# ML200/RoyalTracer-DX

Measured on AMD Instinct MI355X. Metric: Mrays/s + ms/frame at 1080p, 8-bounce Cornell Box, higher is better.
Workload: dtype f32; 1 GPU; cornell_1080p_64spp_8b; scene=generated: Cornell Box (32 triangles, 2 emissive), width=1920, height=1080, spp=64, max_bounces=8, nee_samples=1, rr_start=3, flags=1, triangles=32, parallelism=pixel-tiles/1, tile_size=64

## Files before the change

royaltracer-dx_amd/csrc/rtx_dev_common.hpp:

```cpp
#pragma once
#include "rtx_kernels.hpp"

namespace rtx {

constexpr int kBlock = 256;
constexpr uint32_t kMaxNee = 16;

__device__ __forceinline__ uint32_t lane_id() { return __builtin_amdgcn_mbcnt_hi(~0u, __builtin_amdgcn_mbcnt_lo(~0u, 0u)); }

__device__ __forceinline__ uint32_t block_push(bool pred, uint32_t* lds_counter) {
    const unsigned long long mask = __ballot(pred);
    const uint32_t cnt = (uint32_t)__popcll(mask);
    if (cnt == 0) return 0xFFFFFFFFu;
    const uint32_t prefix = __builtin_amdgcn_mbcnt_hi((uint32_t)(mask >> 32), __builtin_amdgcn_mbcnt_lo((uint32_t)mask, 0u));
    uint32_t base = 0;
    if (lane_id() == 0) base = atomicAdd(lds_counter, cnt);
    base = (uint32_t)__builtin_amdgcn_readfirstlane((int)base);
    return base + prefix;
}

__device__ __forceinline__ bool slot_to_pixel(const DevFrame& f, uint32_t pl, uint32_t& x, uint32_t& y) {
    const uint32_t ts2 = 2u * f.tile_shift;
    const uint32_t k = pl >> ts2, r = pl & ((1u << ts2) - 1u);
    uint32_t tx, ty;
    if (!shard_tile(f, k, tx, ty)) return false;
    const uint32_t bshift = f.tile_shift - 3u;
    const uint32_t blk = r >> 6, ln = r & 63u;
    const uint32_t bx = blk & ((1u << bshift) - 1u), by = blk >> bshift;
    x = (tx << f.tile_shift) + bx * 8u + (ln & 7u);
    y = (ty << f.tile_shift) + by * 8u + (ln >> 3);
    return x < f.width && y < f.height;
}

template <bool LIST> __device__ __forceinline__ uint32_t real_slot(const DevFrame& f, uint32_t v) {
    if constexpr (LIST) return f.list[v >> 8] * (uint32_t)kBlock + (v & 255u);
    else return v;
}
__device__ __forceinline__ bool chunk_image_index(const DevFrame& f, uint32_t lc, uint32_t& gi) {
    const uint32_t cs = 2u * f.tile_shift - 8u;
    uint32_t tx, ty;
    if (!shard_tile(f, lc >> cs, tx, ty)) return false;
    gi = ((ty * f.tiles_x + tx) << cs) | (lc & ((1u << cs) - 1u));
    return true;
}

__device__ __forceinline__ void primary_ray(const CameraGPU& cam, uint32_t W, uint32_t H, uint32_t x, uint32_t y, float jx, float jy, f3& o, f3& d) {
    const float dx = (((float)x + jx) / (float)W) * 2.0f - 1.0f;
    const float dy = (((float)y + jy) / (float)H) * 2.0f - 1.0f;
    const float* P = cam.projI; const float* Vi = cam.viewI;
    const float ndy = -dy;
    f3 tg = mk3(P[0] * dx + P[4] * ndy + P[8] + P[12], P[1] * dx + P[5] * ndy + P[9] + P[13], P[2] * dx + P[6] * ndy + P[10] + P[14]);
    d = normalize(xform_dir(Vi, tg));
    o = mk3(Vi[12], Vi[13], Vi[14]);
}

static_assert(sizeof(CameraGPU) == 64 * sizeof(float), "stage_camera copies one float per lane of the first wave");
__device__ __forceinline__ void stage_camera(CameraGPU& cam, const CameraGPU* __restrict__ cam_p) {
    if (threadIdx.x < 64) ((float*)&cam)[threadIdx.x] = ((const float*)cam_p)[threadIdx.x];
}

__device__ __forceinline__ bool dealt_chunk(const DevFrame& f, uint32_t k, uint32_t& row0, uint32_t nchunks, uint32_t& c) {
    const uint32_t nk = f.taper_levels ? taper_row_width(k, gridDim.x, f.taper_levels) : gridDim.x;
    uint32_t pos = blockIdx.x;
    if (f.taper_levels && blockIdx.x < nk) { pos += (k * 2654435761u) % nk; if (pos >= nk) pos -= nk; }
    c = row0 + pos;
    row0 += nk;
    return !(blockIdx.x >= nk || c >= nchunks);
}

}
```

royaltracer-dx_amd/csrc/rtx_k_bounce_small.hpp:

```cpp
#pragma once
#include "rtx_shade.hpp"

namespace rtx {

template <int WAVES, int HAVE_HIT, bool LAMBERT, bool RING>
__global__ __launch_bounds__(kBlock, WAVES) void k_bounce_small(DevScene sc, const SmallRecPair* __restrict__ small, DevFrame f_in, DevPaths p,
                                                         uint32_t bounce_first, uint32_t bounce_end,
                                                         uint32_t* __restrict__ queue_a, uint32_t* __restrict__ queue_b ,
                                                         uint32_t* __restrict__ qrows ,
                                                         uint32_t* __restrict__ srows ,
                                                         const uint32_t* __restrict__ order ,
                                                         const F4* __restrict__ prim_rec ) {
    extern __shared__ F4 lds[];
    __shared__ uint32_t s_cnt[1 + kMaxNee];
    DevFrame f = f_in;
    f.flags = LAMBERT ? (f_in.flags | 1u) : (f_in.flags & ~1u);
    const uint32_t qid = order ? order[blockIdx.x] : blockIdx.x;
#ifdef RTX_WAVE_CLOCK
    #define RTX_WAVE_STAMP_B(K) do { const uint32_t w_ = blockIdx.x * (kBlock / 64u) + (threadIdx.x >> 6); if (!HAVE_HIT && lane_id() == 0 && w_ < 65536u) g_wgt[2u * w_ + (K)] = __builtin_amdgcn_s_memrealtime(); } while (0)
    RTX_WAVE_STAMP_B(0u);
#endif
    __shared__ F4 s_sho[kBlock], s_shd[kBlock];
    __shared__ uint32_t s_shn[2];
    __shared__ uint8_t s_occ[kBlock];
    if (threadIdx.x <= kMaxNee) s_cnt[threadIdx.x] = 0;
    if (threadIdx.x < 2) s_shn[threadIdx.x] = 0;
#ifndef RTX_NO_SMALL_LDS_TABLES
    constexpr uint32_t kSmallLights = 32, kSmallMats = 16;
    __shared__ F4 s_lt[kSmallLights * 5]; __shared__ float s_ltcdf[kSmallLights]; __shared__ F4 s_mt[kSmallMats * 10];
    const bool lt_lds = sc.nlights && sc.nlights <= kSmallLights, mt_lds = sc.nmat && sc.nmat <= kSmallMats;
    if (lt_lds) { for (uint32_t i = threadIdx.x; i < sc.nlights * 5u; i += kBlock) s_lt[i] = ((const F4*)sc.lights)[i]; if (threadIdx.x < sc.nlights) s_ltcdf[threadIdx.x] = sc.cdf[threadIdx.x]; }
    if (mt_lds) for (uint32_t i = threadIdx.x; i < sc.nmat * 10u; i += kBlock) s_mt[i] = ((const F4*)sc.mats)[i];
    const MatGPU* mats = mt_lds ? (const MatGPU*)s_mt : sc.mats;
    const LightGPU* lds_lights = lt_lds ? (const LightGPU*)s_lt : nullptr; const float* lds_cdf = lt_lds ? s_ltcdf : nullptr;
#else
    const MatGPU* mats = sc.mats; const LightGPU* lds_lights = nullptr; const float* lds_cdf = nullptr;
#endif
    const uint32_t G = gridDim.x;
    uint32_t n = qrows[(size_t)bounce_first * G + qid];
    const uint32_t nee = sc.nlights ? f.nee_samples : 0u;
    const uint32_t nee1 = nee ? nee : 1u;
    const TraceLds L = stage_lds(sc, lds);
    __syncthreads();
    const size_t qb = (size_t)qid * f.qcap;
    uint32_t par = 0;
    constexpr uint32_t kRing = 512u;
    __shared__ uint32_t s_rpid[(HAVE_HIT || !RING) ? 1 : kRing];
    __shared__ F4 s_rhit[(HAVE_HIT || !RING) ? 1 : kRing];
    __shared__ uint32_t s_ring[1], s_rc[3];
    PF_BEGIN;
    for (uint32_t bounce = bounce_first; bounce < bounce_end; bounce++) {
    const bool last = (bounce + 1u == f.max_bounces);
    const float tmin = bounce_tmin(bounce);
    const uint32_t sbounce = HAVE_HIT == 2 ? 0u : bounce;
    const uint32_t* myq = ((bounce & 1u) ? queue_b : queue_a) + qb;
    uint32_t* mynext = ((bounce & 1u) ? queue_a : queue_b) + qb;
    if (!HAVE_HIT && RING) { if (threadIdx.x < 3) s_rc[threadIdx.x] = 0; if (threadIdx.x == 3) s_ring[0] = 0; __syncthreads(); }
    uint32_t next_in = 0;
    uint32_t prod = 0, rk = 0;
    for (uint32_t base = 0; (HAVE_HIT || !RING) ? base < n : true; base += kBlock) {
        PathState S; S.pid = 0; S.o = mk3(0, 0, 0); S.d = mk3(0, 0, 1); S.thr = mk3(0, 0, 0); S.prev_pdf = 1.0f; S.s0 = S.s1 = 0;
        float t = 0.0f, u = 0.0f, v = 0.0f; uint32_t prim = kMissPrim;
        bool active;
        PF_MARK(0);
        Surf sf; sf.mat = 0; sf.normal = mk3(0, 0, 1); sf.pos = mk3(0, 0, 0);
        if (HAVE_HIT == 2) {
            const uint32_t i = base + threadIdx.x;
            active = i < n;
            if (active) {
                S.pid = myq[i];
                const F4 e = p.hit[S.pid];
                const uint32_t pl = f2u(e.x);
                const F4 r0 = prim_rec[pl], r1 = prim_rec[(size_t)f.npl + pl], r2 = prim_rec[(size_t)2 * f.npl + pl], ro = prim_rec[(size_t)3 * f.npl];
                S.s0 = f2u(e.y); S.s1 = f2u(e.z);
                S.o = mk3(ro.x, ro.y, ro.z); S.d = mk3(r0.x, r0.y, r0.z); S.thr = mk3(1.0f, 1.0f, 1.0f); S.prev_pdf = 1.0f;
                sf.pos = mk3(r1.x, r1.y, r1.z); sf.normal = mk3(r2.x, r2.y, r2.z); sf.mat = f2u(r0.w); sf.near_hull = f2u(r1.w) != 0u;
                prim = 0u;
            }
        } else if (HAVE_HIT) {
            const uint32_t i = base + threadIdx.x;
            active = i < n;
            if (active) { S = load_path(p, myq[i]); const F4 h = p.hit[S.pid]; t = h.x; u = h.y; v = h.z; prim = f2u(h.w); }
        } else if (!RING) {
            const uint32_t i = base + threadIdx.x;
            active = i < n;
            if (active) S = load_path(p, myq[i]);
            traverse_small<false>(sc, small, L, S.o, S.d, tmin, active ? kTMax : 0.0f, t, u, v, prim, sc.nsmall, ~0ull, pf, 1);
        } else {
            while (next_in < n && prod - s_ring[0] < kBlock) {
                const uint32_t i = next_in + threadIdx.x;
                const bool act = i < n;
                uint32_t pid = 0; f3 ro = mk3(0, 0, 0), rd = mk3(0, 0, 1);
                if (act) { pid = myq[i]; const F4 a = p.ray_o[pid], b = p.ray_d[pid]; ro = mk3(a.x, a.y, a.z); rd = mk3(b.x, b.y, b.z); }
                float ht, hu, hv; uint32_t hp;
                traverse_small<false>(sc, small, L, ro, rd, tmin, act ? kTMax : 0.0f, ht, hu, hv, hp, sc.nsmall, ~0ull, pf, 1);
                const bool hit = act && hp != kMissPrim;
                const uint32_t slot = prod + block_push(hit, &s_rc[rk]);
                if (hit) { s_rpid[slot & (kRing - 1u)] = pid; s_rhit[slot & (kRing - 1u)] = {ht, hu, hv, u2f(hp)}; }
                next_in += kBlock;
                __syncthreads();
                prod += s_rc[rk];
                if (threadIdx.x == 0) s_rc[rk == 0u ? 2u : rk - 1u] = 0;
                rk = rk == 2u ? 0u : rk + 1u;
            }
            const uint32_t head = s_ring[0], avail = prod - head;
            if (avail == 0u) break;
            const uint32_t take = avail < (uint32_t)kBlock ? avail : (uint32_t)kBlock;
            active = threadIdx.x < take;
            if (active) {
                const uint32_t e = (head + threadIdx.x) & (kRing - 1u);
                S = load_path(p, s_rpid[e]);
                const F4 h = s_rhit[e]; t = h.x; u = h.y; v = h.z; prim = f2u(h.w);
            }
            __syncthreads();
            if (threadIdx.x == 0) s_ring[0] = head + take;
        }
        PF_MARK(2);
        bool shading = false;
        if (active && prim != kMissPrim) {
            PF_COUNT(3);
            if (HAVE_HIT != 2) sf = surface(sc, S.o, S.d, t, u, v, prim);
            if (sf.mat < sc.nmat) {
                const MatGPU& m = mats[sf.mat];
                if (m.Ke_len > 0.0f) add_emissive(sc, p, S, sf, m, sbounce, nee, HAVE_HIT != 0);
                else shading = true;
            } else if (HAVE_HIT) p.rad[S.pid] = {0.0f, 0.0f, 0.0f, 0.0f};
        }
        const f3 outgoing = -S.d, pos = sf.pos;
        const MatGPU* mp = mats + (shading ? sf.mat : 0u);
        f3 normal = sf.normal;
        const float eta_p = LAMBERT ? 0.0f : transmission_eta(*mp, f.flags, outgoing, normal);
        bool loaded = HAVE_HIT && shading; F4 radv = {0, 0, 0, 0};
        PF_MARK(3);
        for (uint32_t j = 0; j < nee; j++) {
            bool push = false;
            F4 so = {0, 0, 0, 0}, sd = {0, 0, 1, 0}; f3 con = mk3(0, 0, 0);
            if (shading) { PF_COUNT(4); push = nee_sample(sc, *mp, f.flags, nee, S, pos, normal, outgoing, so, sd, con, sf.near_hull, eta_p, nullptr, lds_cdf, lds_lights); }
            PF_MARK(4);
            const uint32_t slot = block_push(push, &s_shn[par]);
            if (push) { s_sho[slot] = so; s_shd[slot] = sd; }
            __syncthreads();
            PF_MARK(5);
            const uint32_t ns = s_shn[par];
            if ((threadIdx.x & ~63u) < ns) {
                const bool mine = threadIdx.x < ns;
                const F4 ro = mine ? s_sho[threadIdx.x] : F4{0, 0, 0, 0}, rd = mine ? s_shd[threadIdx.x] : F4{0, 0, 1, 0};
                float st_, su_, sv_; uint32_t sprim;
                const uint32_t nrec_sh = __builtin_amdgcn_ballot_w64(mine && ro.w < 0.0f) != 0ull ? sc.nsmall : sc.nsmall_occ;
                traverse_small<true>(sc, small, L, mk3(ro.x, ro.y, ro.z), mk3(rd.x, rd.y, rd.z), fabsf(ro.w), mine ? rd.w : 0.0f, st_, su_, sv_, sprim, nrec_sh, ~0ull, pf, 6);
                if (mine) s_occ[threadIdx.x] = sprim != kMissPrim ? 1 : 0;
            }
            PF_MARK(7);
            if (threadIdx.x == 0) { s_shn[par ^ 1u] = 0; s_cnt[1 + j] += ns; }
            __syncthreads();
            PF_MARK(8);
            if (push && !s_occ[slot]) {
                if (!loaded) { radv = p.rad[S.pid]; loaded = true; }
                radv.x = radv.x + con.x; radv.y = radv.y + con.y; radv.z = radv.z + con.z;
            }
            par ^= 1u;
        }
        if (loaded) p.rad[S.pid] = radv;
        bool alive = false;
        f3 smp = mk3(0, 0, 1); float P = 0.0f;
        if (shading && !last) { PF_COUNT(9); alive = bsdf_continue(*mp, f, sbounce, S, normal, outgoing, smp, P, eta_p); }
        if (alive) { PF_COUNT(10); store_path(p, S, pos, smp, P); }
        const uint32_t slot = block_push(alive, &s_cnt[0]);
        if (alive) mynext[slot] = S.pid;
        PF_MARK(9);
        if (!HAVE_HIT && RING) __syncthreads();
    }
    __syncthreads();
    n = s_cnt[0];
    if (threadIdx.x == 0) qrows[(size_t)(bounce + 1u) * G + qid] = n;
    if (threadIdx.x >= 1 && threadIdx.x <= nee) srows[((size_t)bounce * nee1 + (threadIdx.x - 1)) * G + qid] = s_cnt[threadIdx.x];
    __syncthreads();
    if (threadIdx.x <= kMaxNee) s_cnt[threadIdx.x] = 0;
    __syncthreads();
    }
    PF_FLUSH;
#ifdef RTX_WAVE_CLOCK
    RTX_WAVE_STAMP_B(1u);
#endif
}

}
```

royaltracer-dx_amd/csrc/rtx_k_film.hpp:

```cpp
#pragma once
#include "rtx_shade.hpp"

namespace rtx {

template <bool LIST>
__global__ __launch_bounds__(kBlock) void k_accumulate(DevFrame f, DevPaths p, F4* __restrict__ accum, AdaptState ad) {
    const uint32_t stride = gridDim.x * kBlock;
    for (uint32_t pl = blockIdx.x * kBlock + threadIdx.x; pl < f.npl; pl += stride) {
        uint32_t x, y;
        if constexpr (LIST) {
            uint32_t gi;
            if ((pl & 255u) == 0u && chunk_image_index(f, f.list[pl >> 8], gi)) ad.count[gi] = ad.count[gi] + f.batch_spp;
        }
        if (!slot_to_pixel(f, real_slot<LIST>(f, pl), x, y)) continue;
        F4 a = accum[(size_t)y * f.width + x];
        F4 h = {0.0f, 0.0f, 0.0f, 0.0f};
        if constexpr (LIST) h = ad.half[(size_t)y * f.width + x];
        for (uint32_t s = 0; s < f.batch_spp; s++) {
            const size_t pid = (size_t)s * f.npl + pl;
            F4 r = {0.0f, 0.0f, 0.0f, 0.0f};
            if (!p.hitmask || ((p.hitmask[pid >> 6] >> (pl & 63u)) & 1ull)) r = p.rad[pid];
            const f3 rv = mk3(r.x, r.y, r.z);
            if (finite3(rv)) {
                a.x = a.x + rv.x; a.y = a.y + rv.y; a.z = a.z + rv.z; a.w = a.w + 1.0f;
                if constexpr (LIST) if ((f.sample_first + s) & 1u) { h.x = h.x + rv.x; h.y = h.y + rv.y; h.z = h.z + rv.z; h.w = h.w + 1.0f; }
            }
        }
        accum[(size_t)y * f.width + x] = a;
        if constexpr (LIST) ad.half[(size_t)y * f.width + x] = h;
    }
}

__global__ __launch_bounds__(kBlock) void k_srgb8(const F4* __restrict__ accum, uint32_t npix, uint32_t* __restrict__ out) {
    const uint32_t i = blockIdx.x * kBlock + threadIdx.x;
    if (i >= npix) return;
    const F4 a = accum[i];
    const float cnt = maxf_(a.w, 1.0f);
    float c[3] = {a.x / cnt, a.y / cnt, a.z / cnt};
    if (is_nan(c[0]) || is_nan(c[1]) || is_nan(c[2])) { c[0] = 1.0f; c[1] = 0.0f; c[2] = 1.0f; }
    if (is_inf(c[0]) || is_inf(c[1]) || is_inf(c[2])) { c[0] = 0.0f; c[1] = 1.0f; c[2] = 1.0f; }
    uint32_t px = 0xFF000000u;
    for (int k = 0; k < 3; k++) {
        float v = c[k] <= 0.0031308f ? 12.92f * c[k] : 1.055f * pow_(c[k], 1.0f / 2.4f) - 0.055f;
        v = saturate(v);
        px |= ((uint32_t)(int)(v * 255.0f + 0.5f)) << (8 * k);
    }
    out[i] = px;
}

__device__ __forceinline__ uint32_t hash_colour(uint32_t id) {
    uint32_t h = id * 2654435761u + 0x9E3779B9u; h ^= h >> 15; h *= 0x85EBCA6Bu; h ^= h >> 13;
    return 0xFF000000u | (0x404040u + (h & 0x00BFBFBFu));
}
__device__ __forceinline__ uint32_t pack_rgb8(float r, float g, float b) {
    const float c[3] = {saturate(r), saturate(g), saturate(b)};
    uint32_t px = 0xFF000000u;
    for (int k = 0; k < 3; k++) px |= ((uint32_t)(int)(c[k] * 255.0f + 0.5f)) << (8 * k);
    return px;
}
__global__ __launch_bounds__(kBlock) void k_debug_layer(DevScene sc, const SmallRecPair* __restrict__ small, uint32_t width, uint32_t height, const CameraGPU* __restrict__ cam, uint32_t layer, uint32_t* __restrict__ out) {
    extern __shared__ F4 lds[];
    const TraceLds L = stage_lds(sc, lds);
    __syncthreads();
    const uint32_t stride = gridDim.x * kBlock;
    for (uint32_t i = blockIdx.x * kBlock + threadIdx.x; i < width * height; i += stride) {
        const uint32_t x = i % width, y = i / width;
        f3 o, d; primary_ray(*cam, width, height, x, y, 0.0f, 0.0f, o, d);
        float t, u, v; uint32_t prim;
        trace_ray<false>(sc, small, L, o, d, kTMinCam, kTMax, t, u, v, prim);
        uint32_t px = 0xFF000000u;
        if (prim != kMissPrim && layer >= 10u && layer <= 17u) {
            const Surf sf = surface(sc, o, d, t, u, v, prim);
            const bool hm = sf.mat < sc.nmat;
            const MatGPU& m = sc.mats[hm ? sf.mat : 0u];
            switch (layer) {
            case 10u: px = pack_rgb8(sf.normal.x * 0.5f + 0.5f, sf.normal.y * 0.5f + 0.5f, sf.normal.z * 0.5f + 0.5f); break;
            case 11u: { const float z = t / (1.0f + t); px = pack_rgb8(z, z, z); break; }
            case 12u: px = hash_colour(sf.mat); break;
            case 13u: px = hm ? pack_rgb8(m.Kd[0], m.Kd[1], m.Kd[2]) : px; break;
            case 14u: px = hash_colour(sf.inst + 0x51ED27u); break;
            case 15u: px = pack_rgb8(1.0f - u - v, u, v); break;
            case 16u: px = hm ? pack_rgb8(m.Ke[0] / (1.0f + m.Ke[0]), m.Ke[1] / (1.0f + m.Ke[1]), m.Ke[2] / (1.0f + m.Ke[2])) : px; break;
            default: px = hm ? pack_rgb8(m.Pr, m.Pm, m.alpha) : px; break;
            }
        }
        out[i] = px;
    }
}

__global__ __launch_bounds__(kBlock) void k_pack_tiles(DevFrame f, const F4* __restrict__ accum, F4* __restrict__ slab) {
    const uint32_t stride = gridDim.x * kBlock;
    for (uint32_t pl = blockIdx.x * kBlock + threadIdx.x; pl < f.npl; pl += stride) {
        uint32_t x, y;
        F4 v = {0, 0, 0, 0};
        if (slot_to_pixel(f, pl, x, y)) v = accum[(size_t)y * f.width + x];
        slab[pl] = v;
    }
}
__global__ __launch_bounds__(kBlock) void k_unpack_tiles(DevFrame f, uint32_t nshards, const F4* __restrict__ slabs, F4* __restrict__ accum) {
    const uint32_t stride = gridDim.x * kBlock;
    const uint32_t total = f.npl * nshards;
    for (uint32_t i = blockIdx.x * kBlock + threadIdx.x; i < total; i += stride) {
        DevFrame g = f; g.shard_rank = i / f.npl; g.shard_count = nshards;
        uint32_t x, y;
        if (slot_to_pixel(g, i - g.shard_rank * f.npl, x, y)) accum[(size_t)y * f.width + x] = slabs[i];
    }
}

}
```

royaltracer-dx_amd/csrc/rtx_k_raygen.hpp:

```cpp
#pragma once
#include "rtx_shade.hpp"

namespace rtx {

template <bool LIST>
__global__ __launch_bounds__(kBlock) void k_raygen(DevFrame f, DevPaths p, const CameraGPU* __restrict__ cam_p, uint32_t* __restrict__ queue, uint32_t* __restrict__ qcount, uint32_t compact) {
    __shared__ CameraGPU cam;
    __shared__ uint32_t s_n;
    stage_camera(cam, cam_p);
    if (threadIdx.x == 0) s_n = 0;
    __syncthreads();
    uint32_t* myq = queue + (size_t)blockIdx.x * f.qcap;
    const uint32_t nchunks = f.chunks_per_sample * f.batch_spp;
    for (uint32_t k = 0, row0 = 0, c; row0 < nchunks; k++) {
        if (!dealt_chunk(f, k, row0, nchunks, c)) continue;
        uint32_t sl = c / f.chunks_per_sample, cl = c - sl * f.chunks_per_sample;
        uint32_t pl = cl * kBlock + threadIdx.x;
        if (f.interleave) {
            const uint32_t sh = f.interleave, S = 1u << sh;
            const uint32_t per = S * f.chunks_per_sample, sg = c / per, r = c - sg * per;
            sl = sg * S + (threadIdx.x & (S - 1u));
            pl = r * (kBlock >> sh) + (threadIdx.x >> sh);
        }
        const uint32_t pid = sl * f.npl + pl;
        uint32_t x = 0, y = 0;
        const bool valid = slot_to_pixel(f, real_slot<LIST>(f, pl), x, y);
        const uint32_t slot = block_push(valid, &s_n);
        if (valid) {
            uint32_t s0, s1; seed_init(x, y, f.sample_first + sl, f.frame_seed, s0, s1);
            float jx = 0.0f, jy = 0.0f;
            if (f.flags & 2u) { jx = tea_next(s0, s1); jy = tea_next(s0, s1); }
            f3 o, d; primary_ray(cam, f.width, f.height, x, y, jx, jy, o, d);
            const uint32_t dst = compact ? blockIdx.x * f.qcap + slot : pid;
            p.ray_o[dst] = {o.x, o.y, o.z, u2f(s1)};
            p.ray_d[dst] = {d.x, d.y, d.z, 1.0f};
            p.thr[dst] = {1.0f, 1.0f, 1.0f, u2f(s0)};
            p.rad[pid] = {0.0f, 0.0f, 0.0f, 0.0f};
            myq[slot] = pid;
        }
    }
    __syncthreads();
    if (threadIdx.x == 0) qcount[blockIdx.x] = s_n;
}

__global__ __launch_bounds__(kBlock) void k_packet_masks(DevScene sc, DevFrame f, const CameraGPU* __restrict__ cam_p, unsigned long long* __restrict__ masks) {
    __shared__ CameraGPU cam;
    stage_camera(cam, cam_p);
    __syncthreads();
    const uint32_t blk = blockIdx.x * (kBlock / 64u) + (threadIdx.x >> 6);
    if (blk >= f.npl / 64u) return;
    uint32_t x = 0, y = 0;
    (void)slot_to_pixel(f, blk * 64u, x, y);
    const unsigned long long keep = packet_keep_mask(sc, cam, f, x & ~7u, y & ~7u);
    if (lane_id() == 0) masks[blk] = keep;
}

template <bool LIST>
__global__ __launch_bounds__(kBlock) void k_raygen_trace_small(DevScene sc, const SmallRecPair* __restrict__ small, DevFrame f, DevPaths p, const CameraGPU* __restrict__ cam_p,
                                                               uint32_t* __restrict__ queue, uint32_t* __restrict__ qcount, uint32_t* __restrict__ gencount,
                                                               const unsigned long long* __restrict__ masks ) {
    extern __shared__ F4 lds[];
    __shared__ CameraGPU cam;
    __shared__ uint32_t s_n[2];
    stage_camera(cam, cam_p);
    if (threadIdx.x < 2) s_n[threadIdx.x] = 0;
    const TraceLds L = stage_lds(sc, lds);
    __syncthreads();
    uint32_t* myq = queue + (size_t)blockIdx.x * f.qcap;
    uint32_t generated = 0;
    const uint32_t nchunks = f.chunks_per_sample * f.batch_spp;
    for (uint32_t k = 0, row0 = 0; row0 < nchunks; k++) {
        const uint32_t nk = f.taper_levels ? taper_row_width(k, gridDim.x, f.taper_levels) : gridDim.x;
        uint32_t pos = blockIdx.x;
        if (f.taper_levels && blockIdx.x < nk) { pos += (k * 2654435761u) % nk; if (pos >= nk) pos -= nk; }
        const uint32_t c = row0 + pos;
        row0 += nk;
        if (blockIdx.x >= nk || c >= nchunks) continue;
        const uint32_t sl = c / f.chunks_per_sample, cl = c - sl * f.chunks_per_sample;
        const uint32_t pl = real_slot<LIST>(f, cl * kBlock + threadIdx.x);
        const uint32_t pid = sl * f.npl + cl * kBlock + threadIdx.x;
        uint32_t x = 0, y = 0, s0 = 0, s1 = 0;
        const bool valid = slot_to_pixel(f, pl, x, y);
        f3 o = mk3(0, 0, 0), d = mk3(0, 0, 1);
        if (valid) {
            seed_init(x, y, f.sample_first + sl, f.frame_seed, s0, s1);
            float jx = 0.0f, jy = 0.0f;
            if (f.flags & 2u) { jx = tea_next(s0, s1); jy = tea_next(s0, s1); }
            primary_ray(cam, f.width, f.height, x, y, jx, jy, o, d);
            generated++;
        }
        const unsigned long long km = masks[pl >> 6];
        const unsigned long long keep = ((unsigned long long)(uint32_t)__builtin_amdgcn_readfirstlane((int)(uint32_t)(km >> 32)) << 32) | (uint32_t)__builtin_amdgcn_readfirstlane((int)(uint32_t)km);
        float t, u, v; uint32_t prim;
        traverse_small<false>(sc, small, L, o, d, kTMinCam, valid ? kTMax : 0.0f, t, u, v, prim, sc.nsmall, keep);
        const bool hit = valid && prim != kMissPrim;
        const unsigned long long hm = __ballot(hit);
        if (lane_id() == 0) p.hitmask[pid >> 6] = hm;
        if (hit) {
            if (f.max_bounces == 0u) p.rad[pid] = {0.0f, 0.0f, 0.0f, 0.0f};
            p.ray_o[pid] = {o.x, o.y, o.z, u2f(s1)};
            p.ray_d[pid] = {d.x, d.y, d.z, 1.0f};
            p.thr[pid] = {1.0f, 1.0f, 1.0f, u2f(s0)};
            p.hit[pid] = {t, u, v, u2f(prim)};
        }
        const uint32_t slot = block_push(hit, &s_n[0]);
        if (hit) myq[slot] = pid;
    }
    atomicAdd(&s_n[1], generated);
    __syncthreads();
    if (threadIdx.x == 0) { qcount[blockIdx.x] = s_n[0]; gencount[blockIdx.x] = s_n[1]; }
}

__global__ __launch_bounds__(kBlock) void k_primary_surface(DevScene sc, const SmallRecPair* __restrict__ small, DevFrame f, const CameraGPU* __restrict__ cam_p,
                                                            unsigned long long* __restrict__ masks, unsigned long long* __restrict__ hits, F4* __restrict__ rec) {
    extern __shared__ F4 lds[];
    __shared__ CameraGPU cam;
    stage_camera(cam, cam_p);
    const TraceLds L = stage_lds(sc, lds);
    __syncthreads();
    const uint32_t pl = blockIdx.x * kBlock + threadIdx.x;
    if (pl >= f.npl) return;
    uint32_t x0 = 0, y0 = 0, x = 0, y = 0;
    (void)slot_to_pixel(f, pl & ~63u, x0, y0);
    const unsigned long long keep = packet_keep_mask(sc, cam, f, x0 & ~7u, y0 & ~7u);
    const bool valid = slot_to_pixel(f, pl, x, y);
    f3 o = mk3(0, 0, 0), d = mk3(0, 0, 1);
    if (valid) primary_ray(cam, f.width, f.height, x, y, 0.0f, 0.0f, o, d);
    float t, u, v; uint32_t prim;
    traverse_small<false>(sc, small, L, o, d, kTMinCam, valid ? kTMax : 0.0f, t, u, v, prim, sc.nsmall, keep);
    const bool hit = valid && prim != kMissPrim;
    const unsigned long long hm = __ballot(hit);
    if (lane_id() == 0) { masks[pl >> 6] = keep; hits[pl >> 6] = hm; }
    if (pl == 0) rec[(size_t)3 * f.npl] = {cam.viewI[12], cam.viewI[13], cam.viewI[14], 0.0f};
    if (hit) {
        const Surf sf = surface(sc, o, d, t, u, v, prim);
        rec[pl] = {d.x, d.y, d.z, u2f(sf.mat)};
        rec[(size_t)f.npl + pl] = {sf.pos.x, sf.pos.y, sf.pos.z, u2f(sf.near_hull ? 1u : 0u)};
        rec[(size_t)2 * f.npl + pl] = {sf.normal.x, sf.normal.y, sf.normal.z, 0.0f};
    }
}

template <bool LIST>
__global__ __launch_bounds__(kBlock) void k_raygen_shared(DevFrame f, DevPaths p, uint32_t* __restrict__ queue, uint32_t* __restrict__ qcount, uint32_t* __restrict__ gencount,
                                                          const unsigned long long* __restrict__ hits ) {
    __shared__ uint32_t s_n[2];
    if (threadIdx.x < 2) s_n[threadIdx.x] = 0;
    __syncthreads();
    uint32_t* myq = queue + (size_t)blockIdx.x * f.qcap;
    uint32_t generated = 0;
    const uint32_t nchunks = f.chunks_per_sample * f.batch_spp;
    for (uint32_t k = 0, row0 = 0, c; row0 < nchunks; k++) {
        if (!dealt_chunk(f, k, row0, nchunks, c)) continue;
        const uint32_t sl = c / f.chunks_per_sample, cl = c - sl * f.chunks_per_sample;
        const uint32_t pl = real_slot<LIST>(f, cl * kBlock + threadIdx.x);
        const uint32_t pid = sl * f.npl + cl * kBlock + threadIdx.x;
        uint32_t x = 0, y = 0;
        if (slot_to_pixel(f, pl, x, y)) generated++;
        const unsigned long long hm = hits[pl >> 6];
        const bool hit = ((hm >> (pl & 63u)) & 1ull) != 0ull;
        if (lane_id() == 0) p.hitmask[pid >> 6] = hm;
        if (hit) {
            if (f.max_bounces == 0u) p.rad[pid] = {0.0f, 0.0f, 0.0f, 0.0f};
            uint32_t s0, s1; seed_init(x, y, f.sample_first + sl, f.frame_seed, s0, s1);
            p.hit[pid] = {u2f(pl), u2f(s0), u2f(s1), 0.0f};
        }
        const uint32_t slot = block_push(hit, &s_n[0]);
        if (hit) myq[slot] = pid;
    }
    atomicAdd(&s_n[1], generated);
    __syncthreads();
    if (threadIdx.x == 0) { qcount[blockIdx.x] = s_n[0]; gencount[blockIdx.x] = s_n[1]; }
}

}
```

royaltracer-dx_amd/csrc/rtx_kernels.hip:

```cpp
#include <hip/hip_runtime.h>
#include <type_traits>
#include "rtx_kernels.hpp"
#include "rtx_dev_common.hpp"
#include "rtx_traverse.hpp"
#include "rtx_shade.hpp"
#include "rtx_restir.hpp"
#include "rtx_restir_wave.hpp"

namespace rtx {

#ifdef RTX_PROFILE_SECTIONS
__device__ unsigned long long g_sec[36];
#define PF_BEGIN Prof pfv; pfv.begin(); Prof* pf = &pfv
#define PF_MARK(i) pf->mark(i)
#define PF_COUNT(i) pf->count(i)
#define PF_FLUSH do { if (lane_id() == 0) for (int i = 0; i < 12; i++) { atomicAdd(&g_sec[i], pfv.acc[i]); atomicAdd(&g_sec[12 + i], pfv.lanes[i]); atomicAdd(&g_sec[24 + i], pfv.calls[i]); } } while (0)
#else
#define PF_BEGIN Prof* pf = nullptr; (void)pf
#define PF_MARK(i) do { } while (0)
#define PF_COUNT(i) do { } while (0)
#define PF_FLUSH do { } while (0)
#endif

}

#include "rtx_k_raygen.hpp"
#include "rtx_k_trace.hpp"
#include "rtx_k_shade.hpp"
#include "rtx_k_bounce_small.hpp"
#include "rtx_k_bounce_bvh.hpp"
#include "rtx_k_film.hpp"
#include "rtx_k_adaptive.hpp"
#include "rtx_k_denoise.hpp"
#include "rtx_k_dbg.hpp"

namespace rtx {

static inline uint32_t grid_for(uint32_t items, uint32_t max_blocks) {
    uint32_t b = (items + kBlock - 1) / kBlock;
    if (b < 1) b = 1;
    return b < max_blocks ? b : max_blocks;
}
static inline size_t small_planes_bytes(const DevScene& sc) { return sc.nsmall ? (size_t)small_planes_count(sc.nsmall) * 16 : 0; }
size_t trace_lds_bytes(const DevScene& sc) {
    return (size_t)sc.lds_nodes * 80 + (size_t)sc.lds_tris * 48 + small_planes_bytes(sc) + (size_t)sc.stack_depth * kBlock * kStackEntryBytes;
}
size_t trace_lds_bytes_queue(const DevScene& sc) {
    const size_t stack = sc.stack_private == 1 ? 0 : (size_t)sc.stack_depth * kBlock * kStackEntryBytes;
    return (size_t)sc.lds_nodes * 80 + (size_t)sc.lds_tris * 48 + small_planes_bytes(sc) + stack;
}

int trace_workgroups_per_cu(const DevScene& sc) {
    int a = 0, b = 0;
    if (hipOccupancyMaxActiveBlocksPerMultiprocessor(&a, k_trace_closest<0, false, 6>, (int)kBlock, trace_lds_bytes(sc)) != hipSuccess) return 0;
    if (hipOccupancyMaxActiveBlocksPerMultiprocessor(&b, k_trace_shadow<0, false, 6>, (int)kBlock, trace_lds_bytes(sc)) != hipSuccess) return 0;
    return a < b ? a : b;
}
void launch_raygen(hipStream_t st, const DevFrame& f, const DevPaths& p, const CameraGPU* cam, uint32_t* queue, uint32_t* qcount, bool compact) {
    if (f.list) hipLaunchKernelGGL(k_raygen<true>, dim3(f.nblocks), dim3(kBlock), 0, st, f, p, cam, queue, qcount, compact ? 1u : 0u);
    else hipLaunchKernelGGL(k_raygen<false>, dim3(f.nblocks), dim3(kBlock), 0, st, f, p, cam, queue, qcount, compact ? 1u : 0u);
}
void launch_packet_masks(hipStream_t st, const DevScene& sc, const DevFrame& f, const CameraGPU* cam, unsigned long long* masks) {
    const uint32_t nblk = f.npl / 64u;
    hipLaunchKernelGGL(k_packet_masks, dim3((nblk + 3u) / 4u), dim3(kBlock), 0, st, sc, f, cam, masks);
}
void launch_raygen_trace_small(hipStream_t st, const DevScene& sc, const DevFrame& f, const DevPaths& p, const CameraGPU* cam, uint32_t* queue, uint32_t* qcount, uint32_t* gencount, const unsigned long long* masks) {
    if (f.list) hipLaunchKernelGGL(k_raygen_trace_small<true>, dim3(f.nblocks), dim3(kBlock), trace_lds_bytes(sc), st, sc, sc.small, f, p, cam, queue, qcount, gencount, masks);
    else hipLaunchKernelGGL(k_raygen_trace_small<false>, dim3(f.nblocks), dim3(kBlock), trace_lds_bytes(sc), st, sc, sc.small, f, p, cam, queue, qcount, gencount, masks);
}
void launch_primary_surface(hipStream_t st, const DevScene& sc, const DevFrame& f, const CameraGPU* cam, unsigned long long* masks, unsigned long long* hits, F4* rec) {
    hipLaunchKernelGGL(k_primary_surface, dim3(f.npl / kBlock), dim3(kBlock), trace_lds_bytes(sc), st, sc, sc.small, f, cam, masks, hits, rec);
}
void launch_raygen_shared(hipStream_t st, const DevFrame& f, const DevPaths& p, uint32_t* queue, uint32_t* qcount, uint32_t* gencount, const unsigned long long* hits) {
    if (f.list) hipLaunchKernelGGL(k_raygen_shared<true>, dim3(f.nblocks), dim3(kBlock), 0, st, f, p, queue, qcount, gencount, hits);
    else hipLaunchKernelGGL(k_raygen_shared<false>, dim3(f.nblocks), dim3(kBlock), 0, st, f, p, queue, qcount, gencount, hits);
}
template <int V> using IntC = std::integral_constant<int, V>;
template <bool V> using BoolC = std::integral_constant<bool, V>;
template <class Launch>
static void launch_trace_variant(const DevFrame& f, const DevScene& sc, uint32_t* heads, uint32_t merge, Launch launch) {
    if (sc.nsmall) heads = nullptr;
    if (heads || sc.nsmall || merge < 1u) merge = 1u;
    if (merge > kMaxMerge) merge = kMaxMerge;
    const uint32_t grid = (f.nblocks + merge - 1u) / merge;
    const bool sched6 = sc.trace_sched == 6u && !sc.nsmall && !sc.trace_cnt;
    auto go = [&](auto stk, auto steal, auto sched, size_t lds_bytes) { launch(stk, steal, sched, grid, lds_bytes, heads, merge); };
    if (sc.stack_private == 1) { if (heads) go(IntC<1>{}, BoolC<true>{}, IntC<-1>{}, trace_lds_bytes_queue(sc)); else go(IntC<1>{}, BoolC<false>{}, IntC<-1>{}, trace_lds_bytes_queue(sc)); }
    else if (sc.stack_ovf) {
        if (heads) go(IntC<2>{}, BoolC<true>{}, IntC<-1>{}, trace_lds_bytes(sc));
        else if (sched6) go(IntC<2>{}, BoolC<false>{}, IntC<6>{}, trace_lds_bytes(sc));
        else go(IntC<2>{}, BoolC<false>{}, IntC<-1>{}, trace_lds_bytes(sc));
    }
    else if (heads) go(IntC<0>{}, BoolC<true>{}, IntC<-1>{}, trace_lds_bytes(sc));
#ifndef RTX_NO_SCHED_SPECIAL
    else if (sched6) go(IntC<0>{}, BoolC<false>{}, IntC<6>{}, trace_lds_bytes(sc));
#endif
    else go(IntC<0>{}, BoolC<false>{}, IntC<-1>{}, trace_lds_bytes(sc));
}
void launch_trace_closest(hipStream_t st, const DevFrame& f, const DevScene& sc, const DevPaths& p, uint32_t bounce, const uint32_t* queue, const uint32_t* qcount, uint32_t* heads, uint32_t merge) {
    const float tmin = bounce == 0 ? kTMinCam : kSBias;
    launch_trace_variant(f, sc, heads, merge, [&](auto stk, auto steal, auto sched, uint32_t grid, size_t lds_bytes, uint32_t* hd, uint32_t mg) {
        hipLaunchKernelGGL((k_trace_closest<decltype(stk)::value, decltype(steal)::value, decltype(sched)::value>), dim3(grid), dim3(kBlock), lds_bytes, st,
                           sc, sc.small, p, queue, qcount, f.qcap, tmin, sc.refill_min, sc.trace_sched, hd, f.nblocks, mg);
    });
}
void launch_bounce_small(hipStream_t st, const DevScene& sc, const DevFrame& f, const DevPaths& p, uint32_t bounce_first, uint32_t bounce_end,
                         uint32_t* queue_a, uint32_t* queue_b, uint32_t* qrows, uint32_t* srows, const uint32_t* order, bool ring, const F4* prim_rec) {
    const bool lam = (f.flags & 1u) != 0u, have_hit = bounce_first == 0u;
#define RTX_LAUNCH_BOUNCE(HH, LL, RR) hipLaunchKernelGGL((k_bounce_small<4, HH, LL, RR>), dim3(f.nblocks), dim3(kBlock), trace_lds_bytes(sc), st, sc, sc.small, f, p, bounce_first, bounce_end, queue_a, queue_b, qrows, srows, order, prim_rec)
    if (have_hit && prim_rec) { if (lam) RTX_LAUNCH_BOUNCE(2, true, false); else RTX_LAUNCH_BOUNCE(2, false, false); }
    else if (have_hit) { if (lam) RTX_LAUNCH_BOUNCE(1, true, false); else RTX_LAUNCH_BOUNCE(1, false, false); }
    else if (ring) { if (lam) RTX_LAUNCH_BOUNCE(0, true, true); else RTX_LAUNCH_BOUNCE(0, false, true); }
    else { if (lam) RTX_LAUNCH_BOUNCE(0, true, false); else RTX_LAUNCH_BOUNCE(0, false, false); }
#undef RTX_LAUNCH_BOUNCE
}
void launch_bounce_bvh(hipStream_t st, const DevScene& sc, const DevFrame& f, const DevPaths& p, uint32_t bounce_first, uint32_t bounce_end,
                       uint32_t* queue_a, uint32_t* queue_b, uint32_t* hitq, uint32_t* qrows, uint32_t* srows, const uint32_t* order) {
    if (sc.stack_private == 1) hipLaunchKernelGGL(k_bounce_bvh<1>, dim3(f.nblocks), dim3(kBlock), trace_lds_bytes_queue(sc), st, sc, f, p, bounce_first, bounce_end, queue_a, queue_b, hitq, qrows, srows, order);
    else if (sc.stack_ovf) hipLaunchKernelGGL(k_bounce_bvh<2>, dim3(f.nblocks), dim3(kBlock), trace_lds_bytes(sc), st, sc, f, p, bounce_first, bounce_end, queue_a, queue_b, hitq, qrows, srows, order);
    else hipLaunchKernelGGL(k_bounce_bvh<0>, dim3(f.nblocks), dim3(kBlock), trace_lds_bytes(sc), st, sc, f, p, bounce_first, bounce_end, queue_a, queue_b, hitq, qrows, srows, order);
}
void launch_order_queues(hipStream_t st, const uint32_t* qcount, uint32_t G, uint32_t* order) {
    hipLaunchKernelGGL(k_order_queues, dim3(1), dim3(1024), 0, st, qcount, G, order);
}
void launch_trace_shadow(hipStream_t st, const DevFrame& f, const DevScene& sc, const DevPaths& p, uint32_t j, const uint32_t* shcount, uint32_t* heads, uint32_t merge) {
    const size_t seg = (size_t)j * f.qcap * f.nblocks;
    launch_trace_variant(f, sc, heads, merge, [&](auto stk, auto steal, auto sched, uint32_t grid, size_t lds_bytes, uint32_t* hd, uint32_t mg) {
        hipLaunchKernelGGL((k_trace_shadow<decltype(stk)::value, decltype(steal)::value, decltype(sched)::value>), dim3(grid), dim3(kBlock), lds_bytes, st,
                           sc, sc.small, p, p.sh_o + seg, p.sh_d + seg, p.sh_c + seg, shcount, f.qcap, sc.refill_min, sc.trace_sched, hd, f.nblocks, mg);
    });
}
static size_t shade_lds_bytes(const DevScene& sc, bool sort) { uint32_t lb, mb; shade_lds_plan(sc.nlights, sc.nmat, sort, lb, mb); return (size_t)lb + mb; }
void launch_shade(hipStream_t st, const DevScene& sc, const DevFrame& f, const DevPaths& p, uint32_t bounce,
                  const uint32_t* queue, const uint32_t* qcount, uint32_t* next_queue, uint32_t* next_count, uint32_t* shcounts) {
#define RTX_LAUNCH_SHADE(SS, LL) hipLaunchKernelGGL((k_shade<SS, LL>), dim3(f.nblocks), dim3(kBlock), shade_lds_bytes(sc, SS), st, sc, f, p, bounce, queue, qcount, next_queue, next_count, shcounts)
    const bool lam = (f.flags & 1u) != 0u;
    if (sc.shade_dense && !sc.sort_materials) {
        if (lam) hipLaunchKernelGGL((k_shade_dense<true>), dim3(f.nblocks), dim3(kBlock), 0, st, sc, f, p, bounce, queue, qcount, next_queue, next_count, shcounts);
        else hipLaunchKernelGGL((k_shade_dense<false>), dim3(f.nblocks), dim3(kBlock), 0, st, sc, f, p, bounce, queue, qcount, next_queue, next_count, shcounts);
    }
    else if (sc.sort_materials) { if (lam) RTX_LAUNCH_SHADE(true, true); else RTX_LAUNCH_SHADE(true, false); }
    else { if (lam) RTX_LAUNCH_SHADE(false, true); else RTX_LAUNCH_SHADE(false, false); }
#undef RTX_LAUNCH_SHADE
}
void launch_v6_pass1(hipStream_t st, uint32_t max_blocks, const DevScene& sc, const DevFrame& f, const CameraGPU* cam, uint32_t sample_id,
                     F4* accum, uint32_t* res_di, uint32_t* res_gi, uint32_t* sdata, unsigned long long* counters, const uint32_t* pixels, uint32_t npixels) {
    hipLaunchKernelGGL(k_v6_pass1, dim3(grid_for(pixels ? npixels : f.npl, max_blocks)), dim3(kBlock), trace_lds_bytes(sc), st, sc, sc.small, f, cam, sample_id, accum, res_di, res_gi, sdata, counters, pixels, npixels);
}
static inline RestirBufs rs_bufs(uint32_t* const* b) { return RestirBufs{b[0], b[1], b[2], b[3], b[4], b[5]}; }
void launch_restir_pass2(hipStream_t st, uint32_t max_blocks, const DevScene& sc, const DevFrame& f, const CameraGPU* cam, uint32_t* const bufs[6], unsigned long long* counters,
                         const uint32_t* pixels, uint32_t npixels) {
    hipLaunchKernelGGL(k_restir_pass2, dim3(grid_for(pixels ? npixels : f.npl, max_blocks)), dim3(kBlock), trace_lds_bytes(sc), st, sc, sc.small, f, cam, rs_bufs(bufs), counters, pixels, npixels);
}
void launch_restir_pack_state(hipStream_t st, uint32_t max_blocks, const DevFrame& f, uint32_t* const bufs[6], uint32_t* slab) {
    hipLaunchKernelGGL(k_restir_pack_state, dim3(grid_for(f.npl, max_blocks)), dim3(kBlock), 0, st, f, rs_bufs(bufs), slab);
}
void launch_restir_unpack_state(hipStream_t st, uint32_t max_blocks, const DevFrame& f, uint32_t nshards, const uint32_t* slabs, uint32_t* const bufs[6]) {
    hipLaunchKernelGGL(k_restir_unpack_state, dim3(grid_for(f.npl * nshards, max_blocks)), dim3(kBlock), 0, st, f, nshards, slabs, rs_bufs(bufs));
}
void launch_restir_halo(hipStream_t st, uint32_t max_blocks, uint32_t width, bool pack, const uint32_t* rects4, uint32_t n, uint32_t* const bufs[6], uint32_t* buf) {
    HaloRects R{}; R.n = n; R.first[0] = 0;
    for (uint32_t k = 0; k < n; k++) { R.x0[k] = rects4[4 * k]; R.y0[k] = rects4[4 * k + 1]; R.w[k] = rects4[4 * k + 2]; R.first[k + 1] = R.first[k] + rects4[4 * k + 2] * rects4[4 * k + 3]; }
    if (!R.first[n]) return;
    if (pack) hipLaunchKernelGGL(k_restir_halo<true>, dim3(grid_for(R.first[n], max_blocks)), dim3(kBlock), 0, st, width, R, rs_bufs(bufs), buf);
    else hipLaunchKernelGGL(k_restir_halo<false>, dim3(grid_for(R.first[n], max_blocks)), dim3(kBlock), 0, st, width, R, rs_bufs(bufs), buf);
}
void launch_restir_pass3(hipStream_t st, uint32_t max_blocks, const DevScene& sc, const DevFrame& f, const CameraGPU* cam, uint32_t* const bufs[6], F4* accum, unsigned long long* counters) {
    hipLaunchKernelGGL(k_restir_pass3, dim3(grid_for(f.npl, max_blocks)), dim3(kBlock), trace_lds_bytes(sc), st, sc, sc.small, f, cam, rs_bufs(bufs), accum, counters);
}
void launch_trace_occ(hipStream_t st, const DevScene& sc_in, const RsQ& q, const uint32_t* shcnt) {
    DevPaths none{};
    DevScene sc = sc_in; sc.any_order = sc_in.any_order_occ;
#define RTX_LAUNCH_TO(CC) hipLaunchKernelGGL((k_trace_shadow<SL_, false, CC, 1>), dim3(q.G), dim3(kBlock), trace_lds_bytes(sc), st, sc, sc.small, none, q.sh_o, q.sh_d, (const F4*)nullptr, shcnt, q.rcap, sc.refill_min, sc.trace_sched, (uint32_t*)nullptr, q.G, 1u, q.sh_pay, q.occ)
    if (sc.stack_ovf) { constexpr int SL_ = 2; if (sc.trace_sched == 6u && !sc.nsmall && !sc.trace_cnt) RTX_LAUNCH_TO(6); else RTX_LAUNCH_TO(-1); }
    else { constexpr int SL_ = 0; if (sc.trace_sched == 6u && !sc.nsmall && !sc.trace_cnt) RTX_LAUNCH_TO(6); else RTX_LAUNCH_TO(-1); }
#undef RTX_LAUNCH_TO
}
void launch_rs_raygen(hipStream_t st, const DevFrame& f, const RsQ& q, const CameraGPU* cam, uint32_t sample_id, uint32_t* cnt_out) {
    hipLaunchKernelGGL(k_rs_raygen, dim3(q.G), dim3(kBlock), 0, st, f, q, cam, sample_id, cnt_out);
}
void launch_rs_p1_ris(hipStream_t st, const DevScene& sc, const DevFrame& f, const RsQ& q, const uint32_t* cnt_in, uint32_t* cnt_out, F4* accum, uint32_t* res_di, uint32_t* res_gi, uint32_t* sdata) {
    hipLaunchKernelGGL(k_rs_p1_ris, dim3(q.G), dim3(kBlock), 0, st, sc, f, q, cnt_in, cnt_out, accum, res_di, res_gi, sdata);
}
void launch_rs_p1_ris_finish(hipStream_t st, const DevScene& sc, const DevFrame& f, const RsQ& q, const uint32_t* cnt_in, uint32_t* cnt_out, uint32_t* shcnt, uint32_t* res_di, uint32_t* sdata) {
    hipLaunchKernelGGL(k_rs_p1_ris_finish, dim3(q.G), dim3(kBlock), 0, st, sc, f, q, cnt_in, cnt_out, shcnt, res_di, sdata);
}
void launch_rs_p1_first(hipStream_t st, const DevScene& sc, const DevFrame& f, const RsQ& q, const uint32_t* cnt_in, uint32_t* cnt_out) {
    hipLaunchKernelGGL(k_rs_p1_first, dim3(q.G), dim3(kBlock), 0, st, sc, f, q, cnt_in, cnt_out);
}
void launch_rs_p1_loop(hipStream_t st, const DevScene& sc, const DevFrame& f, const RsQ& q, uint32_t set, uint32_t iter, const uint32_t* cnt_in, uint32_t* cnt_out) {
    hipLaunchKernelGGL(k_rs_p1_loop, dim3(q.G), dim3(kBlock), 0, st, sc, f, q, set, iter, cnt_in, cnt_out);
}
void launch_rs_p1_emit_final(hipStream_t st, const DevScene& sc, const DevFrame& f, const RsQ& q, const CameraGPU* cam, uint32_t* const* bufs, uint32_t* shcnt) {
    hipLaunchKernelGGL(k_rs_p1_emit_final, dim3(q.G), dim3(kBlock), 0, st, sc, f, q, cam, bufs ? rs_bufs(bufs) : RestirBufs{}, bufs ? 1u : 0u, shcnt);
}
void launch_rs_p1_finish(hipStream_t st, const DevScene& sc, const DevFrame& f, const RsQ& q, F4* accum, uint32_t* res_di, uint32_t* res_gi, uint32_t* sdata, const CameraGPU* cam, uint32_t* const* bufs) {
#ifdef RTX_RS_FUSED_FINISH
    hipLaunchKernelGGL((k_rs_p1_finish<true, true>), dim3(q.G), dim3(kBlock), 0, st, sc, f, q, accum, res_di, res_gi, sdata, cam, bufs ? rs_bufs(bufs) : RestirBufs{}, bufs ? 1u : 0u);
#else
    hipLaunchKernelGGL((k_rs_p1_finish<true, false>), dim3(q.G), dim3(kBlock), 0, st, sc, f, q, accum, res_di, res_gi, sdata, cam, RestirBufs{}, 0u);
    if (bufs) hipLaunchKernelGGL((k_rs_p1_finish<false, true>), dim3(q.G), dim3(kBlock), 0, st, sc, f, q, accum, res_di, res_gi, sdata, cam, rs_bufs(bufs), 1u);
#endif
}
void launch_rs_p3_keys(hipStream_t st, const DevFrame& f, const RsQ& q, uint32_t* const bufs[6], F4* key_a, F4* key_b) {
    hipLaunchKernelGGL(k_rs_p3_keys, dim3(q.G), dim3(kBlock), 0, st, f, q, rs_bufs(bufs), RsKeys{key_a, key_b});
}
void launch_rs_p3_select(hipStream_t st, const DevScene& sc, const DevFrame& f, const RsQ& q, const CameraGPU* cam, uint32_t* const bufs[6], uint32_t* shcnt, F4* key_a, F4* key_b) {
    if (key_a) { hipLaunchKernelGGL(k_rs_p3_select_keys, dim3(q.G), dim3(kBlock), 0, st, sc, f, q, cam, rs_bufs(bufs), RsKeys{key_a, key_b}, shcnt); return; }
    hipLaunchKernelGGL(k_rs_p3_select, dim3(q.G), dim3(kBlock), 0, st, sc, f, q, cam, rs_bufs(bufs), shcnt);
}
void launch_rs_p3_merge(hipStream_t st, const DevScene& sc, const DevFrame& f, const RsQ& q, uint32_t* const bufs[6], uint32_t* shcnt) {
    hipLaunchKernelGGL(k_rs_p3_merge<false>, dim3(q.G), dim3(kBlock), 0, st, sc, f, q, rs_bufs(bufs), shcnt);
    hipLaunchKernelGGL(k_rs_p3_merge<true>, dim3(q.G), dim3(kBlock), 0, st, sc, f, q, rs_bufs(bufs), shcnt);
}
void launch_rs_p3_shade(hipStream_t st, const DevScene& sc, const DevFrame& f, const RsQ& q, uint32_t* const bufs[6], F4* accum) {
    hipLaunchKernelGGL(k_rs_p3_shade, dim3(q.G), dim3(kBlock), 0, st, sc, f, q, rs_bufs(bufs), accum);
}
void launch_accumulate(hipStream_t st, uint32_t max_blocks, const DevFrame& f, const DevPaths& p, F4* accum) {
    hipLaunchKernelGGL(k_accumulate<false>, dim3(grid_for(f.npl, max_blocks)), dim3(kBlock), 0, st, f, p, accum, AdaptState{});
}
void launch_accumulate_list(hipStream_t st, uint32_t max_blocks, const DevFrame& f, const DevPaths& p, F4* accum, const AdaptState& ad) {
    hipLaunchKernelGGL(k_accumulate<true>, dim3(grid_for(f.npl, max_blocks)), dim3(kBlock), 0, st, f, p, accum, ad);
}
void launch_adaptive_error(hipStream_t st, const DevFrame& f, const F4* accum, const AdaptState& ad, float threshold, float dark_floor) {
    hipLaunchKernelGGL(k_adaptive_error, dim3(f.chunks_per_sample), dim3(kBlock), 0, st, f, accum, ad, threshold, dark_floor);
}
void launch_adaptive_compact(hipStream_t st, const DevFrame& f, const AdaptState& ad, uint32_t max_spp, uint32_t* list, uint32_t* out5) {
    hipLaunchKernelGGL(k_adaptive_compact, dim3(1), dim3(kCompactBlock), 0, st, f, ad, max_spp, list, out5);
}
void launch_denoise_guides(hipStream_t st, uint32_t max_blocks, const DevScene& sc, uint32_t width, uint32_t height, const CameraGPU* cam, F4* guides) {
    hipLaunchKernelGGL(k_denoise_guides, dim3(grid_for(width * height, max_blocks)), dim3(kBlock), trace_lds_bytes(sc), st, sc, sc.small, width, height, cam, guides);
}
uint32_t denoise_workgroups(uint32_t width, uint32_t height) { return ((width + kDnTileW - 1u) / kDnTileW) * ((height + kDnTileH - 1u) / kDnTileH); }
void launch_denoise_level(hipStream_t st, DenoiseLevel a, const F4* in, const F4* guides, F4* out, uint32_t* partial, bool staged) {
    a.tiles_x = (a.width + kDnTileW - 1u) / kDnTileW;
    const dim3 grid(denoise_workgroups(a.width, a.height));
#define RTX_LAUNCH_DN(SS, FF) hipLaunchKernelGGL((k_denoise_level<SS, FF>), grid, dim3(kBlock), 0, st, a, in, guides, out, partial)
    if (a.first) { if (staged && a.step == 1u) RTX_LAUNCH_DN(1, true); else RTX_LAUNCH_DN(0, true); }
    else if (staged && a.step == 2u) RTX_LAUNCH_DN(2, false);
    else if (staged && a.step == 4u) RTX_LAUNCH_DN(4, false);
    else RTX_LAUNCH_DN(0, false);
#undef RTX_LAUNCH_DN
}
void launch_denoise_count(hipStream_t st, const uint32_t* partial, uint32_t n, uint32_t* out) {
    hipLaunchKernelGGL(k_denoise_count, dim3(1), dim3(kBlock), 0, st, partial, n, out);
}
void launch_srgb8(hipStream_t st, const F4* accum, uint32_t npix, uint32_t* out) {
    hipLaunchKernelGGL(k_srgb8, dim3((npix + kBlock - 1) / kBlock), dim3(kBlock), 0, st, accum, npix, out);
}
void launch_debug_layer(hipStream_t st, uint32_t max_blocks, const DevScene& sc, uint32_t width, uint32_t height, const CameraGPU* cam, uint32_t layer, uint32_t* out) {
    hipLaunchKernelGGL(k_debug_layer, dim3(grid_for(width * height, max_blocks)), dim3(kBlock), trace_lds_bytes(sc), st, sc, sc.small, width, height, cam, layer, out);
}
void launch_pack_tiles(hipStream_t st, uint32_t max_blocks, const DevFrame& f, const F4* accum, F4* slab) {
    hipLaunchKernelGGL(k_pack_tiles, dim3(grid_for(f.npl, max_blocks)), dim3(kBlock), 0, st, f, accum, slab);
}
void launch_unpack_tiles(hipStream_t st, uint32_t max_blocks, const DevFrame& f, uint32_t nshards, const F4* slabs, F4* accum) {
    hipLaunchKernelGGL(k_unpack_tiles, dim3(grid_for(f.npl * nshards, max_blocks)), dim3(kBlock), 0, st, f, nshards, slabs, accum);
}
void launch_dbg_trace(hipStream_t st, const DevScene& sc, const F4* rays, uint32_t n, int any, F4* hits) {
    hipLaunchKernelGGL(k_dbg_trace, dim3(grid_for(n, 2048)), dim3(kBlock), trace_lds_bytes(sc), st, sc, sc.small, rays, n, any, hits);
}
void launch_dbg_surface(hipStream_t st, const DevScene& sc, const F4* rays, const F4* hits, uint32_t n, F4* out) {
    hipLaunchKernelGGL(k_dbg_surface, dim3((n + kBlock - 1) / kBlock), dim3(kBlock), 0, st, sc, rays, hits, n, out);
}
void launch_dbg_bsdf_eval(hipStream_t st, const DevScene& sc, uint32_t mat, uint32_t flags, const float* in9, uint32_t n, float* out8) {
    hipLaunchKernelGGL(k_dbg_bsdf_eval, dim3((n + kBlock - 1) / kBlock), dim3(kBlock), 0, st, sc, mat, flags, in9, n, out8);
}
void launch_dbg_bsdf_sample(hipStream_t st, const DevScene& sc, uint32_t mat, uint32_t flags, const float* in8, uint32_t n, float* out8) {
    hipLaunchKernelGGL(k_dbg_bsdf_sample, dim3((n + kBlock - 1) / kBlock), dim3(kBlock), 0, st, sc, mat, flags, in8, n, out8);
}
void launch_dbg_tea(hipStream_t st, uint32_t s0, uint32_t s1, uint32_t n, float* out, uint32_t* seed_out) {
    hipLaunchKernelGGL(k_dbg_tea, dim3(1), dim3(64), 0, st, s0, s1, n, out, seed_out);
}
void launch_dbg_primary(hipStream_t st, const DevFrame& f, const CameraGPU* cam, uint32_t sample_id, F4* rays) {
    hipLaunchKernelGGL(k_dbg_primary, dim3((f.width * f.height + kBlock - 1) / kBlock), dim3(kBlock), 0, st, f, cam, sample_id, rays);
}

}

#ifdef RTX_PROFILE_SECTIONS
extern "C" int rtx_debug_traversal(unsigned long long* out8, int reset) {
    if (hipDeviceSynchronize() != hipSuccess) return -1;
    if (out8 && hipMemcpyFromSymbol(out8, HIP_SYMBOL(rtx::g_trv), sizeof(unsigned long long) * 8) != hipSuccess) return -1;
    if (reset) { unsigned long long z[8] = {0}; if (hipMemcpyToSymbol(HIP_SYMBOL(rtx::g_trv), z, sizeof(z)) != hipSuccess) return -1; }
    return 0;
}
extern "C" int rtx_debug_sections(unsigned long long* out36, int reset) {
    if (hipDeviceSynchronize() != hipSuccess) return -1;
    if (out36 && hipMemcpyFromSymbol(out36, HIP_SYMBOL(rtx::g_sec), sizeof(unsigned long long) * 36) != hipSuccess) return -1;
    if (reset) { unsigned long long z[36] = {0}; if (hipMemcpyToSymbol(HIP_SYMBOL(rtx::g_sec), z, sizeof(z)) != hipSuccess) return -1; }
    return 0;
}
#endif

#ifdef RTX_WAVE_CLOCK
extern "C" int rtx_debug_wave_times(unsigned long long* out, unsigned nwaves, int reset) {
    if (hipDeviceSynchronize() != hipSuccess || nwaves > 65536u) return -1;
    if (out && hipMemcpyFromSymbol(out, HIP_SYMBOL(rtx::g_wgt), sizeof(unsigned long long) * 2 * nwaves) != hipSuccess) return -1;
    if (reset) { void* d = nullptr; if (hipGetSymbolAddress(&d, HIP_SYMBOL(rtx::g_wgt)) != hipSuccess || hipMemset(d, 0, sizeof(unsigned long long) * 2 * 65536) != hipSuccess) return -1; }
    return 0;
}
#endif
```

royaltracer-dx_amd/csrc/rtx_kernels.hpp:

```cpp
#pragma once
#include <hip/hip_runtime.h>
#include "rtx_types.hpp"

namespace rtx {

struct DevScene {
    const Node8GPU* nodes;  uint32_t nnodes;
    const F4* nodes_f; uint32_t node_v4;
    const TriGPU*   tris;   uint32_t ntris;
    const TriShade* shade;
    const SmallRecPair* small; uint32_t nsmall;
    uint32_t nsmall_occ;
    const F4* small_poly;
    const TriGPU* small_tris;
    float small_cm, small_delta;
    const MatGPU*   mats;   uint32_t nmat;
    const InstGPU*  insts;  uint32_t ninst;
    const LightGPU* lights; uint32_t nlights;
    const float* cdf;
    float total_weight;
    uint32_t lds_nodes, lds_tris;
    uint32_t stack_depth;
    unsigned long long* stack_ovf; uint32_t stack_ovf_stride;
    uint32_t stack_private;
    uint32_t sort_materials;
    uint32_t refill_min, trace_sched;
    uint32_t shade_dense;
    uint32_t any_order;
    float cell_o[3], cell_s[3]; uint32_t cell_bits;
    uint32_t any_order_occ;
    unsigned long long* trace_cnt;
    uint32_t occluder_cache;
};

struct DevFrame {
    uint32_t width, height;
    uint32_t tile_size, tile_shift, tiles_x, tiles_y;
    uint32_t shard_rank, shard_count;
    uint32_t blk_gx, blk_gy;
    uint32_t npl;
    uint32_t batch_spp;
    uint32_t sample_first;
    uint32_t max_bounces, nee_samples, rr_start, frame_seed, flags;
    uint32_t nblocks, qcap, chunks_per_sample;
    uint32_t interleave;
    uint32_t taper_levels;
    uint32_t hist_x0, hist_y0, hist_x1, hist_y1; unsigned long long* hist_stale;
    const uint32_t* list;
};

#if defined(__HIPCC__)
#define RTX_TAPER_HD __host__ __device__ __forceinline__
#else
#define RTX_TAPER_HD inline
#endif
RTX_TAPER_HD uint32_t taper_row_width(uint32_t k, uint32_t G, uint32_t levels) {
    const uint32_t m = k & ((1u << (levels - 1u)) - 1u);
    if (m == 0u) return G;
    uint32_t lg = 0; while ((m >> (lg + 1u)) != 0u) lg++;
    return G - (G >> (levels - 1u - lg));
}
#if defined(__HIPCC__)
#define RTX_TILE_HD __host__ __device__ __forceinline__
#else
#define RTX_TILE_HD inline
#endif
RTX_TILE_HD bool shard_tile(const DevFrame& f, uint32_t k, uint32_t& tx, uint32_t& ty) {
    if (f.blk_gx) {
        const uint32_t bx = f.shard_rank % f.blk_gx, by = f.shard_rank / f.blk_gx;
        const uint32_t tx0 = bx * f.tiles_x / f.blk_gx, tx1 = (bx + 1u) * f.tiles_x / f.blk_gx, ty0 = by * f.tiles_y / f.blk_gy, ty1 = (by + 1u) * f.tiles_y / f.blk_gy;
        const uint32_t bw = (f.tiles_x + f.blk_gx - 1u) / f.blk_gx;
        tx = tx0 + k % bw; ty = ty0 + k / bw;
        return tx < tx1 && ty < ty1;
    }
    const uint32_t t = f.shard_rank + k * f.shard_count;
    if (t >= f.tiles_x * f.tiles_y) return false;
    ty = t / f.tiles_x; tx = t - ty * f.tiles_x;
    return true;
}

struct DevPaths {
    F4* ray_o;
    F4* ray_d;
    F4* thr;
    F4* rad;
    F4* hit;
    unsigned long long* hitmask;
    F4* sh_o;
    F4* sh_d;
    F4* sh_c;
    F4* out_o; F4* out_d; F4* out_thr;
    uint8_t* oct_out; const uint8_t* oct_in; uint32_t* perm; uint32_t key_mode;
};

constexpr uint32_t kMaxMerge = 8;
constexpr uint32_t kRsStreams = 7;
constexpr uint32_t kRsOcc = 16;
constexpr uint32_t kRsCand = 10;
struct RsQ {
    uint32_t nitems; const uint32_t* pixels;
    uint32_t G, qcap, rcap;
    F4* st[2][kRsStreams];
    F4* hit;
    uint32_t* cls;
    F4* fin;
    F4* cold;
    uint8_t* occ;
    uint32_t* cand;
    F4* sh_o; F4* sh_d; uint32_t* sh_pay;
    unsigned long long* rays;
};

size_t trace_lds_bytes(const DevScene& sc);
int trace_workgroups_per_cu(const DevScene& sc);
void launch_raygen(hipStream_t, const DevFrame&, const DevPaths&, const CameraGPU* cam, uint32_t* queue, uint32_t* qcount, bool compact);
void launch_trace_closest(hipStream_t, const DevFrame&, const DevScene&, const DevPaths&, uint32_t bounce, const uint32_t* queue, const uint32_t* qcount, uint32_t* heads, uint32_t merge = 1);
void launch_packet_masks(hipStream_t, const DevScene&, const DevFrame&, const CameraGPU* cam, unsigned long long* masks);
void launch_raygen_trace_small(hipStream_t, const DevScene&, const DevFrame&, const DevPaths&, const CameraGPU* cam, uint32_t* queue, uint32_t* qcount, uint32_t* gencount, const unsigned long long* masks);
void launch_primary_surface(hipStream_t, const DevScene&, const DevFrame&, const CameraGPU* cam, unsigned long long* masks, unsigned long long* hits, F4* rec);
void launch_raygen_shared(hipStream_t, const DevFrame&, const DevPaths&, uint32_t* queue, uint32_t* qcount, uint32_t* gencount, const unsigned long long* hits);
void launch_bounce_small(hipStream_t, const DevScene&, const DevFrame&, const DevPaths&, uint32_t bounce_first, uint32_t bounce_end,
                         uint32_t* queue_a, uint32_t* queue_b, uint32_t* qrows, uint32_t* srows, const uint32_t* order, bool ring = true,
                         const F4* prim_rec = nullptr);
void launch_bounce_bvh(hipStream_t, const DevScene&, const DevFrame&, const DevPaths&, uint32_t bounce_first, uint32_t bounce_end,
                       uint32_t* queue_a, uint32_t* queue_b, uint32_t* hitq, uint32_t* qrows, uint32_t* srows, const uint32_t* order);
void launch_order_queues(hipStream_t, const uint32_t* qcount, uint32_t G, uint32_t* order);
void launch_trace_shadow(hipStream_t, const DevFrame&, const DevScene&, const DevPaths&, uint32_t j, const uint32_t* shcount, uint32_t* heads, uint32_t merge = 1);
void launch_shade(hipStream_t, const DevScene&, const DevFrame&, const DevPaths&, uint32_t bounce,
                  const uint32_t* queue, const uint32_t* qcount, uint32_t* next_queue, uint32_t* next_count, uint32_t* shcounts);
void launch_v6_pass1(hipStream_t, uint32_t max_blocks, const DevScene&, const DevFrame&, const CameraGPU* cam, uint32_t sample_id,
                     F4* accum, uint32_t* res_di, uint32_t* res_gi, uint32_t* sdata, unsigned long long* counters, const uint32_t* pixels = nullptr, uint32_t npixels = 0);
void launch_restir_pass2(hipStream_t, uint32_t max_blocks, const DevScene&, const DevFrame&, const CameraGPU* cam, uint32_t* const bufs[6], unsigned long long* counters,
                         const uint32_t* pixels = nullptr, uint32_t npixels = 0);
void launch_restir_pack_state(hipStream_t, uint32_t max_blocks, const DevFrame&, uint32_t* const bufs[6], uint32_t* slab);
void launch_restir_unpack_state(hipStream_t, uint32_t max_blocks, const DevFrame&, uint32_t nshards, const uint32_t* slabs, uint32_t* const bufs[6]);
constexpr uint32_t kHaloPeers = 16;
void launch_restir_halo(hipStream_t, uint32_t max_blocks, uint32_t width, bool pack, const uint32_t* rects4 , uint32_t n , uint32_t* const bufs[6], uint32_t* buf);
void launch_restir_pass3(hipStream_t, uint32_t max_blocks, const DevScene&, const DevFrame&, const CameraGPU* cam, uint32_t* const bufs[6], F4* accum, unsigned long long* counters);
void launch_trace_occ(hipStream_t, const DevScene&, const RsQ&, const uint32_t* shcnt);
void launch_rs_raygen(hipStream_t, const DevFrame&, const RsQ&, const CameraGPU* cam, uint32_t sample_id, uint32_t* cnt_out);
void launch_rs_p1_ris(hipStream_t, const DevScene&, const DevFrame&, const RsQ&, const uint32_t* cnt_in, uint32_t* cnt_out, F4* accum, uint32_t* res_di, uint32_t* res_gi, uint32_t* sdata);
void launch_rs_p1_ris_finish(hipStream_t, const DevScene&, const DevFrame&, const RsQ&, const uint32_t* cnt_in, uint32_t* cnt_out, uint32_t* shcnt, uint32_t* res_di, uint32_t* sdata);
void launch_rs_p1_first(hipStream_t, const DevScene&, const DevFrame&, const RsQ&, const uint32_t* cnt_in, uint32_t* cnt_out);
void launch_rs_p1_loop(hipStream_t, const DevScene&, const DevFrame&, const RsQ&, uint32_t set, uint32_t iter, const uint32_t* cnt_in, uint32_t* cnt_out);
void launch_rs_p1_emit_final(hipStream_t, const DevScene&, const DevFrame&, const RsQ&, const CameraGPU* cam, uint32_t* const* bufs, uint32_t* shcnt);
void launch_rs_p1_finish(hipStream_t, const DevScene&, const DevFrame&, const RsQ&, F4* accum, uint32_t* res_di, uint32_t* res_gi, uint32_t* sdata, const CameraGPU* cam, uint32_t* const* bufs);
void launch_rs_p3_keys(hipStream_t, const DevFrame&, const RsQ&, uint32_t* const bufs[6], F4* key_a, F4* key_b);
void launch_rs_p3_select(hipStream_t, const DevScene&, const DevFrame&, const RsQ&, const CameraGPU* cam, uint32_t* const bufs[6], uint32_t* shcnt, F4* key_a = nullptr, F4* key_b = nullptr);
void launch_rs_p3_merge(hipStream_t, const DevScene&, const DevFrame&, const RsQ&, uint32_t* const bufs[6], uint32_t* shcnt);
void launch_rs_p3_shade(hipStream_t, const DevScene&, const DevFrame&, const RsQ&, uint32_t* const bufs[6], F4* accum);
void launch_accumulate(hipStream_t, uint32_t max_blocks, const DevFrame&, const DevPaths&, F4* accum);
struct AdaptState { F4* half; uint32_t* count; uint32_t* flag; };
void launch_accumulate_list(hipStream_t, uint32_t max_blocks, const DevFrame&, const DevPaths&, F4* accum, const AdaptState&);
void launch_adaptive_error(hipStream_t, const DevFrame&, const F4* accum, const AdaptState&, float threshold, float dark_floor);
void launch_adaptive_compact(hipStream_t, const DevFrame&, const AdaptState&, uint32_t max_spp, uint32_t* list, uint32_t* out5);
struct DenoiseLevel { uint32_t width, height, tiles_x, step, normal_power_log2, first, last; float inv_sigma_plane, inv_sigma_color_s; };
void launch_denoise_guides(hipStream_t, uint32_t max_blocks, const DevScene&, uint32_t width, uint32_t height, const CameraGPU* cam, F4* guides);
uint32_t denoise_workgroups(uint32_t width, uint32_t height);
void launch_denoise_level(hipStream_t, DenoiseLevel, const F4* in, const F4* guides, F4* out, uint32_t* partial, bool staged);
void launch_denoise_count(hipStream_t, const uint32_t* partial, uint32_t n, uint32_t* out);
void launch_srgb8(hipStream_t, const F4* accum, uint32_t npix, uint32_t* out);
void launch_debug_layer(hipStream_t, uint32_t max_blocks, const DevScene&, uint32_t width, uint32_t height, const CameraGPU* cam, uint32_t layer, uint32_t* out);
void launch_pack_tiles(hipStream_t, uint32_t max_blocks, const DevFrame&, const F4* accum, F4* slab);
void launch_unpack_tiles(hipStream_t, uint32_t max_blocks, const DevFrame&, uint32_t nshards, const F4* slabs, F4* accum);
void launch_refit(hipStream_t, Node8GPU* nodes, const uint32_t* level_start, uint32_t nlevels, TriGPU* tris, uint32_t ntris, const TriShade* shade,
                  const InstGPU* insts, const F4* objtris, F4* node_aabb, uint32_t* scale_bits,
                  const uint32_t* moved = nullptr, uint8_t* tri_dirty = nullptr, uint8_t* node_dirty = nullptr,
                  const uint32_t* hidden = nullptr);
uint32_t tree_cost_partials(uint32_t nnodes);
void launch_tree_cost(hipStream_t, const F4* node_aabb, uint32_t nnodes, float* partial);
void launch_dbg_trace(hipStream_t, const DevScene&, const F4* rays, uint32_t n, int any, F4* hits);
void launch_dbg_surface(hipStream_t, const DevScene&, const F4* rays, const F4* hits, uint32_t n, F4* out);
void launch_dbg_bsdf_eval(hipStream_t, const DevScene&, uint32_t mat, uint32_t flags, const float* in9, uint32_t n, float* out8);
void launch_dbg_bsdf_sample(hipStream_t, const DevScene&, uint32_t mat, uint32_t flags, const float* in8, uint32_t n, float* out8);
void launch_dbg_tea(hipStream_t, uint32_t s0, uint32_t s1, uint32_t n, float* out, uint32_t* seed_out);
void launch_dbg_primary(hipStream_t, const DevFrame&, const CameraGPU* cam, uint32_t sample_id, F4* rays);

}
```

royaltracer-dx_amd/csrc/rtx_math.hpp:

```cpp
#pragma once
#include <stdint.h>
#include <math.h>
#include <string.h>

#if defined(__HIPCC__)
#include <hip/hip_runtime.h>
#define RTX_HD __host__ __device__ __forceinline__
#else
#define RTX_HD inline
#endif

namespace rtx {

constexpr float kPI      = 3.1415f;
constexpr float kInvPI   = 1.0f / kPI;
constexpr float kSBias   = 0.00002f;
constexpr float kEps     = 0.000001f;
constexpr float kTwoPi   = 6.28318548202514648f;
constexpr float kTMinCam = 0.0001f;
constexpr float kTMax    = 10000.0f;
constexpr uint32_t kMissPrim = 0xFFFFFFFFu;
constexpr uint32_t kMissMat  = 0xFFFFFFFEu;

struct f3 { float x, y, z; };

RTX_HD f3 mk3(float x, float y, float z) { f3 r; r.x = x; r.y = y; r.z = z; return r; }
RTX_HD f3 operator+(f3 a, f3 b) { return mk3(a.x + b.x, a.y + b.y, a.z + b.z); }
RTX_HD f3 operator-(f3 a, f3 b) { return mk3(a.x - b.x, a.y - b.y, a.z - b.z); }
RTX_HD f3 operator-(f3 a) { return mk3(-a.x, -a.y, -a.z); }
RTX_HD f3 operator*(f3 a, float s) { return mk3(a.x * s, a.y * s, a.z * s); }
RTX_HD float dot(f3 a, f3 b) { return __builtin_fmaf(a.z, b.z, __builtin_fmaf(a.y, b.y, a.x * b.x)); }
RTX_HD f3 cross(f3 a, f3 b) { return mk3(__builtin_fmaf(a.y, b.z, -(a.z * b.y)), __builtin_fmaf(a.z, b.x, -(a.x * b.z)), __builtin_fmaf(a.x, b.y, -(a.y * b.x))); }
RTX_HD f3 madd3(f3 a, float s, f3 b) { return mk3(__builtin_fmaf(a.x, s, b.x), __builtin_fmaf(a.y, s, b.y), __builtin_fmaf(a.z, s, b.z)); }
RTX_HD f3 lincomb3(f3 x, float a, f3 y, float b, f3 z, float c) {
    return mk3(__builtin_fmaf(z.x, c, __builtin_fmaf(y.x, b, x.x * a)), __builtin_fmaf(z.y, c, __builtin_fmaf(y.y, b, x.y * a)), __builtin_fmaf(z.z, c, __builtin_fmaf(y.z, b, x.z * a)));
}
RTX_HD float length(f3 a) { return sqrtf(dot(a, a)); }
#ifndef RTX_DET_REL
#define RTX_DET_REL 1.52587890625e-05f
#endif
constexpr float kDetRel = RTX_DET_REL;
RTX_HD float tri_det_floor(f3 e1, f3 e2) { return kDetRel * (sqrtf(dot(e1, e1)) * sqrtf(dot(e2, e2))); }
RTX_HD uint32_t f2u(float f);
RTX_HD float u2f(uint32_t u);
RTX_HD float rsqrt_det(float x) {
    float y = u2f(0x5f375a86u - (f2u(x) >> 1));
    const float h = 0.5f * x;
    y = y * __builtin_fmaf(-h, y * y, 1.5f);
    y = y * __builtin_fmaf(-h, y * y, 1.5f);
    return __builtin_fmaf(0.5f * y, __builtin_fmaf(-x, y * y, 1.0f), y);
}
RTX_HD f3 normalize(f3 a) { return a * rsqrt_det(dot(a, a)); }
RTX_HD float saturate(float x) { return x < 0.0f ? 0.0f : (x > 1.0f ? 1.0f : x); }
RTX_HD float maxf_(float a, float b) { return a > b ? a : b; }
RTX_HD float minf_(float a, float b) { return a < b ? a : b; }
RTX_HD bool is_nan(float x) { return x != x; }
RTX_HD bool is_inf(float x) { return fabsf(x) == INFINITY; }
RTX_HD bool finite3(f3 a) { return !(is_nan(a.x) || is_nan(a.y) || is_nan(a.z) || is_inf(a.x) || is_inf(a.y) || is_inf(a.z)); }
RTX_HD bool is_zero3(f3 a) { return a.x == 0.0f && a.y == 0.0f && a.z == 0.0f; }

RTX_HD f3 safe_mul(float s, f3 v) { f3 r = v * s; return finite3(r) ? r : mk3(0.0f, 0.0f, 0.0f); }
RTX_HD float safe_mul(float s, float v) { float r = s * v; return (is_nan(r) || is_inf(r)) ? 0.0f : r; }

RTX_HD uint32_t f2u(float f) {
#if defined(__HIP_DEVICE_COMPILE__)
    return __float_as_uint(f);
#else
    uint32_t u; memcpy(&u, &f, 4); return u;
#endif
}
RTX_HD float u2f(uint32_t u) {
#if defined(__HIP_DEVICE_COMPILE__)
    return __uint_as_float(u);
#else
    float f; memcpy(&f, &u, 4); return f;
#endif
}

RTX_HD float tea_next(uint32_t& s0, uint32_t& s1) {
    uint32_t v0 = s0, v1 = s1, sum = 0u;
#pragma unroll
    for (int i = 0; i < 4; i++) {
        sum += 0x9e3779b9u;
        v0 += ((v1 << 4) + 0xA341316Cu) ^ (v1 + sum) ^ ((v1 >> 5) + 0xC8013EA4u);
        v1 += ((v0 << 4) + 0xAD90777Du) ^ (v0 + sum) ^ ((v0 >> 5) + 0x7E95761Eu);
    }
    s0 = v0; s1 = v1;
    return (float)v0 * (1.0f / 4294967296.0f);
}
RTX_HD void seed_init(uint32_t x, uint32_t y, uint32_t s, uint32_t frame_seed, uint32_t& s0, uint32_t& s1) {
    s0 = (y * 73856093u) ^ (x * 19349663u) ^ (s * 83492791u) ^ (frame_seed * 293803u);
    s1 = (x * 37623481u) ^ (y * 51964263u) ^ (s * 68250729u) ^ (frame_seed * 423977u);
}

RTX_HD void sincos_(float x, float& sn, float& cs) {
    int j = (int)(x * 1.27323954473516f);
    j = (j + 1) & ~1;
    float y = (float)j;
    float r = ((x - y * 0.78515625f) - y * 2.4187564849853515625e-4f) - y * 3.77489497744594108e-8f;
    float z = r * r;
    float ps = ((-1.9515295891e-4f * z + 8.3321608736e-3f) * z - 1.6666654611e-1f) * z * r + r;
    float pc = ((2.443315711809948e-5f * z - 1.388731625493765e-3f) * z + 4.166664568298827e-2f) * z * z - 0.5f * z + 1.0f;
    int q = (j >> 1) & 3;
    float a = (q & 1) ? pc : ps;
    float b = (q & 1) ? ps : pc;
    sn = (q & 2) ? -a : a;
    cs = (q == 1 || q == 2) ? -b : b;
}

RTX_HD float pow_(float x, float y) {
    if (!(x > 0.0f)) return 0.0f;
    uint32_t ux = f2u(x);
    int e = (int)((ux >> 23) & 0xFF) - 127;
    float m = u2f((ux & 0x007FFFFFu) | 0x3F800000u);
    if (m > 1.41421356f) { m = m * 0.5f; e += 1; }
    float t = (m - 1.0f) / (m + 1.0f);
    float t2 = t * t;
    float ln = 2.0f * t * (1.0f + t2 * (0.333333333f + t2 * (0.2f + t2 * (0.142857143f + t2 * 0.111111111f))));
    float l2 = (float)e + ln * 1.44269504089f;
    float p = y * l2;
    if (p < -126.0f) return 0.0f;
    if (p > 127.0f) return INFINITY;
    float fl = floorf(p + 0.5f);
    float f = p - fl;
    float g = f * 0.693147180560f;
    float ex = 1.0f + g * (1.0f + g * (0.5f + g * (0.166666667f + g * (0.0416666667f + g * (0.00833333333f + g * 0.00138888889f)))));
    return ex * u2f((uint32_t)((int)fl + 127) << 23);
}

RTX_HD f3 xform_point(const float* m, f3 p) {
    return mk3(__builtin_fmaf(m[8], p.z, __builtin_fmaf(m[4], p.y, __builtin_fmaf(m[0], p.x, m[12]))),
               __builtin_fmaf(m[9], p.z, __builtin_fmaf(m[5], p.y, __builtin_fmaf(m[1], p.x, m[13]))),
               __builtin_fmaf(m[10], p.z, __builtin_fmaf(m[6], p.y, __builtin_fmaf(m[2], p.x, m[14]))));
}
RTX_HD f3 xform_dir(const float* m, f3 p) {
    return mk3(__builtin_fmaf(m[8], p.z, __builtin_fmaf(m[4], p.y, m[0] * p.x)),
               __builtin_fmaf(m[9], p.z, __builtin_fmaf(m[5], p.y, m[1] * p.x)),
               __builtin_fmaf(m[10], p.z, __builtin_fmaf(m[6], p.y, m[2] * p.x)));
}

}
```

royaltracer-dx_amd/csrc/rtx_render.hip:

```cpp
#include "rtx_ctx.hpp"

namespace {

struct BatchPlan { uint32_t bspp, G, qchunks, taper_levels, max_blocks; bool compact; };

BatchPlan plan_batches(const rtx_ctx* c, uint32_t spp, const DevFrame& f, bool fused_bvh) {
    BatchPlan B{};
    B.bspp = (uint32_t)std::max<uint64_t>(1, std::min<uint64_t>(spp, c->opt.paths_per_batch / f.npl));
    const bool tiny_fused = c->dsc.nsmall && c->opt.fused;
    auto plan = [&](uint32_t spp_batch) {
        const uint32_t nchunks = f.chunks_per_sample * spp_batch;
        const uint32_t bpc_hi = tiny_fused ? 40u : 32u, per_wg = tiny_fused ? 16u : 8u;
        const uint32_t bpc = c->opt.blocks_per_cu ? c->opt.blocks_per_cu
                                                  : std::max<uint32_t>(8u, std::min<uint32_t>(bpc_hi, (nchunks / per_wg + (uint32_t)c->num_cus - 1u) / (uint32_t)c->num_cus));
        B.max_blocks = (uint32_t)c->num_cus * bpc;
        B.G = std::max<uint32_t>(1, std::min<uint32_t>(nchunks, B.max_blocks));
        B.taper_levels = 0; B.qchunks = (nchunks + B.G - 1) / B.G;
        if (c->opt.taper && !fused_bvh && B.G >= 64u && nchunks >= 4u * B.G) {
            B.taper_levels = c->opt.taper_levels;
            B.qchunks = 0;
            for (uint32_t k = 0, row0 = 0; row0 < nchunks; k++) { row0 += taper_row_width(k, B.G, B.taper_levels); B.qchunks++; }
        }
    };
    plan(B.bspp);
    B.compact = c->opt.compact_state && !tiny_fused && !fused_bvh;
    while (B.taper_levels && B.compact && B.bspp > 1u && (uint64_t)B.G * B.qchunks * 256u > c->opt.paths_per_batch) {
        const uint32_t next = (uint32_t)std::max<uint64_t>(1, (uint64_t)B.bspp * c->opt.paths_per_batch / ((uint64_t)B.G * B.qchunks * 256u));
        B.bspp = next < B.bspp ? next : B.bspp - 1u;
        plan(B.bspp);
    }
    return B;
}

struct FrameRun {
    DevPaths P; uint32_t* queue[2]; uint32_t* cnt; const CameraGPU* cam; hipStream_t st;
    const F4* prim_rec;
    uint32_t rec_npl;
    uint32_t G, mb, nee, nee1; bool compact, osort, stealing; size_t hstride, nheads;
    uint32_t* Q(uint32_t b) const { return cnt + (size_t)b * G; }
    uint32_t* S(uint32_t b, uint32_t j) const { return cnt + ((size_t)(mb + 1) + (size_t)b * nee1 + j) * G; }
};

int enqueue_tiny_fused(rtx_ctx* c, const FrameRun& R, const DevFrame& fb) {
    const hipStream_t st = R.st;
    uint32_t* gen_row = R.cnt + ((size_t)(R.mb + 1) + (size_t)R.mb * R.nee1) * R.G;
    if (R.prim_rec) { Timed t(c, RTX_K_RAYGEN); launch_raygen_shared(st, fb, R.P, R.queue[0], R.Q(0), gen_row, (const unsigned long long*)c->pt.d_prim_hits.p); }
    else { Timed t(c, RTX_K_RAYGEN); launch_raygen_trace_small(st, c->dsc, fb, R.P, R.cam, R.queue[0], R.Q(0), gen_row, (const unsigned long long*)c->pt.d_pmask.p); }
    const uint32_t* order = nullptr;
    if (c->opt.lpt_order && R.G > 1) { launch_order_queues(st, R.Q(0), R.G, (uint32_t*)c->pt.d_order.p); order = (const uint32_t*)c->pt.d_order.p; }
    DevFrame f0 = fb; f0.npl = R.rec_npl;
    { Timed t(c, RTX_K_BOUNCE); launch_bounce_small(st, c->dsc, f0, R.P, 0, 1, R.queue[0], R.queue[1], R.Q(0), R.S(0, 0), order, false, R.prim_rec); }
    if (R.mb > 1) { Timed t(c, RTX_K_BOUNCE); launch_bounce_small(st, c->dsc, fb, R.P, 1, R.mb, R.queue[0], R.queue[1], R.Q(0), R.S(0, 0), order, c->opt.bounce_ring); }
    return RTX_OK;
}

int enqueue_fused_bvh(rtx_ctx* c, const FrameRun& R, const DevFrame& fb) {
    const hipStream_t st = R.st;
    { Timed t(c, RTX_K_RAYGEN); launch_raygen(st, fb, R.P, R.cam, R.queue[0], R.Q(0), R.compact); }
    const uint32_t* ord = nullptr;
    if (c->opt.lpt_order && R.G > 1) { launch_order_queues(st, R.Q(0), R.G, (uint32_t*)c->pt.d_order.p); ord = (const uint32_t*)c->pt.d_order.p; }
    Timed t(c, RTX_K_BOUNCE);
    launch_bounce_bvh(st, c->dsc, fb, R.P, 0, R.mb, R.queue[0], R.queue[1], (uint32_t*)c->pt.d_hitq.p, R.Q(0), R.S(0, 0), ord);
    return RTX_OK;
}

int enqueue_bounces(rtx_ctx* c, const FrameRun& R, const DevFrame& fb) {
    const hipStream_t st = R.st; const DevPaths& P = R.P;
    const uint32_t G = R.G, mb = R.mb, nee = R.nee, nee1 = R.nee1; const bool compact = R.compact, osort = R.osort, stealing = R.stealing;
    { Timed t(c, RTX_K_RAYGEN); launch_raygen(st, fb, P, R.cam, R.queue[0], R.Q(0), compact); }
    if (stealing) HIPCHK(c, hipMemsetAsync(c->pt.d_heads.p, 0, R.nheads * 4, st));
    const bool ovl = c->opt.overlap_shadow && !c->opt.timing;
    if (ovl && !c->pt.aux) c->pt.aux = c->streams.set.s[1];
    hipEvent_t ev_shadow_done = nullptr;
    auto Hd = [&](uint32_t b, uint32_t k) { return stealing ? (uint32_t*)c->pt.d_heads.p + ((size_t)b * (1 + nee1) + k) * R.hstride : nullptr; };
    auto merge_for = [&](uint64_t pred_num, bool have) -> uint32_t {
        if (!have || !c->opt.merge_rays || !c->pt.pred_paths || stealing) return 1u;
        const double rays = (double)pred_num * (double)((uint64_t)fb.npl * fb.batch_spp) / (double)c->pt.pred_paths;
        uint32_t k = 1u;
        while (k < kMaxMerge && G / (2u * k) >= (uint32_t)c->num_cus * 8u && rays * k / G < (double)c->opt.merge_rays) k *= 2u;
        return k;
    };
    for (uint32_t b = 0; b < mb; b++) {
        uint32_t* q = R.queue[b & 1]; uint32_t* qn = R.queue[(b + 1) & 1];
        DevPaths Pb = P;
        if (compact) {
            F4* set[2][3] = {{(F4*)c->pt.d_ray_o.p, (F4*)c->pt.d_ray_d.p, (F4*)c->pt.d_thr.p}, {(F4*)c->pt.d_alt_o.p, (F4*)c->pt.d_alt_d.p, (F4*)c->pt.d_alt_thr.p}};
            Pb.ray_o = set[b & 1][0]; Pb.ray_d = set[b & 1][1]; Pb.thr = set[b & 1][2];
            Pb.out_o = set[(b + 1) & 1][0]; Pb.out_d = set[(b + 1) & 1][1]; Pb.out_thr = set[(b + 1) & 1][2];
            if (osort) {
                Pb.oct_out = c->opt.octant_sort == 2 ? nullptr : (uint8_t*)c->pt.d_oct[(b + 1) & 1].p;
                if (b >= (c->opt.octant_sort == 3 ? 2u : 1u)) { Pb.oct_in = (const uint8_t*)c->pt.d_oct[b & 1].p; Pb.perm = (uint32_t*)c->pt.d_perm.p; }
            }
        }
        DevScene scb = c->dsc;
        if (c->scene.wide_nodes && b >= 1u) { scb.nodes_f = (const F4*)c->scene.d_nodes_wide.p; scb.node_v4 = 8u; }
        if (c->scene.lds_nodes_closest) scb.lds_nodes = c->scene.lds_nodes_closest;
        { Timed t(c, RTX_K_TRACE); launch_trace_closest(st, fb, scb, Pb, b, q, R.Q(b), Hd(b, 0), merge_for(b < c->pt.pred_q.size() ? c->pt.pred_q[b] : 0, b < c->pt.pred_q.size())); }
        if (ovl && ev_shadow_done) HIPCHK(c, hipStreamWaitEvent(st, ev_shadow_done, 0));
        { Timed t(c, RTX_K_SHADE); launch_shade(st, c->dsc, fb, Pb, b, q, R.Q(b), qn, R.Q(b + 1), R.S(b, 0)); }
        hipStream_t ss = st;
        if (ovl && nee) {
            hipEvent_t e = c->ev.take(); ev_shadow_done = c->ev.take();
            if (!e || !ev_shadow_done) { c->err = "render: out of events"; return RTX_ERR_HIP; }
            HIPCHK(c, hipEventRecord(e, st)); HIPCHK(c, hipStreamWaitEvent(c->pt.aux, e, 0));
            ss = c->pt.aux;
        }
        for (uint32_t j = 0; j < nee; j++) { const size_t ps = (size_t)b * nee1 + j; Timed t(c, RTX_K_SHADOW, ss); launch_trace_shadow(ss, fb, c->dsc, Pb, j, R.S(b, j), Hd(b, 1 + j), merge_for(ps < c->pt.pred_s.size() ? c->pt.pred_s[ps] : 0, ps < c->pt.pred_s.size() && c->pt.pred_nee1 == nee1)); }
        if (ovl && nee) HIPCHK(c, hipEventRecord(ev_shadow_done, c->pt.aux));
    }
    if (ovl && ev_shadow_done) HIPCHK(c, hipStreamWaitEvent(st, ev_shadow_done, 0));
    return RTX_OK;
}

}

extern "C" {

int rtx_render(rtx_ctx* c, const rtx_params* p) {
    BIND(c);
    if (!c->committed) { c->err = "render: scene not committed"; return RTX_ERR_STATE; }
    if (!c->camera_set) { c->err = "render: camera not set"; return RTX_ERR_STATE; }
    DevFrame f;
    int r = make_frame(c, p, f);
    if (r) return r;
    if (p->max_bounces == 0 || p->max_bounces > 64) { c->err = "params: max_bounces must be in [1, 64]"; return RTX_ERR_INVALID; }
    if (p->nee_samples > 16) { c->err = "params: nee_samples must be <= 16"; return RTX_ERR_INVALID; }
    if ((r = ensure_accum(c, p->width, p->height, false))) return r;
    memset(c->stats.kernel_ms, 0, sizeof(c->stats.kernel_ms));
    memset(c->stats.kernel_launches, 0, sizeof(c->stats.kernel_launches));
    memset(c->stats.kernel_items, 0, sizeof(c->stats.kernel_items));
    c->stats.rays_primary = c->stats.rays_extension = c->stats.rays_shadow = c->stats.paths = c->stats.primary_hits = 0; c->stats.render_ms = 0;
    if (p->spp == 0) return RTX_OK;
    c->ad.pure = false;
    if ((r = render_frame(c, p, f, p->spp, nullptr))) return r;
    if (c->opt.async && !c->own_stream) return RTX_OK;
    return finish_render(c);
}

}

int render_frame(rtx_ctx* c, const rtx_params* p, const DevFrame& f_real, uint32_t spp, const ListPass* lp) {
    int r = RTX_OK;
    DevFrame f = f_real;
    if (lp) { f.list = lp->list; f.npl = lp->n_active * 256u; f.chunks_per_sample = lp->n_active; }
    const uint32_t sample_first = lp ? lp->sample_first : p->sample_base;

    const uint32_t nee = c->dsc.nlights ? p->nee_samples : 0;
    const bool tiny_fused = c->dsc.nsmall && c->opt.fused;
    const bool fused_bvh = !c->dsc.nsmall && c->opt.fused_bvh && c->opt.trace_sched >= 5u;
    const BatchPlan B = plan_batches(c, spp, f, fused_bvh);
    const uint32_t bspp = B.bspp, G = B.G;
    const uint64_t cap64 = (uint64_t)f.npl * bspp;
    if (cap64 > 0x7FFFFFFFull) { c->err = "render: batch too large"; return RTX_ERR_INVALID; }
    const uint32_t cap = (uint32_t)cap64;

    HIPCHK(c, c->pt.d_rad.ensure((size_t)cap * 16));
    const uint32_t qcap = B.qchunks * 256u;
    f.nblocks = G; f.qcap = qcap; f.taper_levels = B.taper_levels;
    const size_t qtot = (size_t)G * qcap;
    const size_t nstate = B.compact ? qtot : (size_t)cap;
    if (nstate > 0xFFFFFFFFull) { c->err = "render: batch too large"; return RTX_ERR_INVALID; }
    HIPCHK(c, c->pt.d_ray_o.ensure(nstate * 16)); HIPCHK(c, c->pt.d_ray_d.ensure(nstate * 16)); HIPCHK(c, c->pt.d_thr.ensure(nstate * 16)); HIPCHK(c, c->pt.d_hit.ensure(nstate * 16));
    if (B.compact) { HIPCHK(c, c->pt.d_alt_o.ensure(nstate * 16)); HIPCHK(c, c->pt.d_alt_d.ensure(nstate * 16)); HIPCHK(c, c->pt.d_alt_thr.ensure(nstate * 16)); }
    HIPCHK(c, c->pt.d_queue[0].ensure(qtot * 4)); HIPCHK(c, c->pt.d_queue[1].ensure(qtot * 4));
    HIPCHK(c, c->pt.d_order.ensure((size_t)G * 4));
    if (fused_bvh) HIPCHK(c, c->pt.d_hitq.ensure(qtot * 4));
    FrameRun R{};
    R.G = G; R.mb = p->max_bounces; R.nee = nee; R.nee1 = std::max<uint32_t>(nee, 1); R.compact = B.compact;
    R.stealing = !c->dsc.nsmall && !fused_bvh && c->opt.work_stealing && p->max_bounces > 0;
    R.hstride = (size_t)G + (G + 31) / 32;
    R.nheads = R.stealing ? (size_t)p->max_bounces * (1 + std::max<uint32_t>(nee, 1)) * R.hstride : 0;
    if (R.stealing) HIPCHK(c, c->pt.d_heads.ensure(R.nheads * 4));
    HIPCHK(c, c->pt.d_pmask.ensure(((size_t)f_real.npl / 64 + 1) * 8));
    const bool shared_primary = tiny_fused && c->opt.shared_primary && !(p->flags & RTX_FLAG_JITTER);
    if (shared_primary) { HIPCHK(c, c->pt.d_prim_rec.ensure(((size_t)f_real.npl * 3 + 1) * 16)); HIPCHK(c, c->pt.d_prim_hits.ensure(((size_t)f_real.npl / 64 + 1) * 8)); }
    R.prim_rec = shared_primary ? (const F4*)c->pt.d_prim_rec.p : nullptr; R.rec_npl = f_real.npl;
    const size_t shn = qtot * R.nee1;
    HIPCHK(c, c->pt.d_sh_o.ensure(shn * 16)); HIPCHK(c, c->pt.d_sh_d.ensure(shn * 16)); HIPCHK(c, c->pt.d_sh_c.ensure(shn * 16));
    DevPaths& P = R.P;
    P.ray_o = (F4*)c->pt.d_ray_o.p; P.ray_d = (F4*)c->pt.d_ray_d.p; P.thr = (F4*)c->pt.d_thr.p; P.rad = (F4*)c->pt.d_rad.p; P.hit = (F4*)c->pt.d_hit.p;
    P.hitmask = nullptr;
    P.out_o = P.out_d = P.out_thr = nullptr; P.oct_out = nullptr; P.oct_in = nullptr; P.perm = nullptr; P.key_mode = (uint32_t)c->opt.octant_sort;
    R.osort = c->opt.octant_sort && B.compact && !R.stealing;
    if (R.osort) { HIPCHK(c, c->pt.d_oct[0].ensure(qtot)); HIPCHK(c, c->pt.d_oct[1].ensure(qtot)); HIPCHK(c, c->pt.d_perm.ensure(qtot * 4)); }
    if (R.osort && c->opt.octant_sort == 2) { HIPCHK(c, hipMemsetAsync(c->pt.d_oct[0].p, 0, qtot, c->stream)); HIPCHK(c, hipMemsetAsync(c->pt.d_oct[1].p, 0, qtot, c->stream)); }
    if (tiny_fused) { HIPCHK(c, c->pt.d_hitmask.ensure(((size_t)cap / 64 + 1) * 8)); P.hitmask = (unsigned long long*)c->pt.d_hitmask.p; }
    P.sh_o = (F4*)c->pt.d_sh_o.p; P.sh_d = (F4*)c->pt.d_sh_d.p; P.sh_c = (F4*)c->pt.d_sh_c.p;
    R.queue[0] = (uint32_t*)c->pt.d_queue[0].p; R.queue[1] = (uint32_t*)c->pt.d_queue[1].p;
    const uint32_t mb = R.mb, nee1 = R.nee1;
    const size_t ncnt = ((size_t)(mb + 1) + (size_t)mb * nee1 + 1) * G;
    const uint32_t nbatches = (spp + bspp - 1) / bspp;
    HIPCHK(c, c->pt.d_counters.ensure(ncnt * 4));
    HIPCHK(c, c->pt.h_counters.ensure(ncnt * nbatches * 4));
    R.cnt = (uint32_t*)c->pt.d_counters.p;
    R.cam = (const CameraGPU*)c->d_cam.p;
    c->ev.used = 0; c->timed.clear();
    const hipStream_t st = R.st = c->stream;

    struct AuxJoin { rtx_ctx* c; bool armed = true; ~AuxJoin() { if (armed && c->pt.aux) (void)hipStreamSynchronize(c->pt.aux); } } aux_join{c};
    HIPCHK(c, hipEventRecord(c->ev.begin, st));
    HIPCHK(c, hipMemsetAsync(R.cnt, 0, ncnt * 4, st));
    const bool tables_in_place = lp && !lp->first;
    if (shared_primary && !tables_in_place) { Timed t(c, RTX_K_RAYGEN); launch_primary_surface(st, c->dsc, f_real, R.cam, (unsigned long long*)c->pt.d_pmask.p, (unsigned long long*)c->pt.d_prim_hits.p, (F4*)c->pt.d_prim_rec.p); }
    else if (tiny_fused && !shared_primary && !tables_in_place) launch_packet_masks(st, c->dsc, f_real, R.cam, (unsigned long long*)c->pt.d_pmask.p);
    for (uint32_t bi = 0; bi < nbatches; bi++) {
        DevFrame fb = f;
        fb.sample_first = sample_first + bi * bspp;
        fb.batch_spp = std::min(bspp, spp - bi * bspp);
        fb.interleave = 0;
        if (c->opt.sample_interleave) while (fb.interleave < 4u && !((fb.batch_spp >> fb.interleave) & 1u)) fb.interleave++;
        r = tiny_fused ? enqueue_tiny_fused(c, R, fb) : fused_bvh ? enqueue_fused_bvh(c, R, fb) : enqueue_bounces(c, R, fb);
        if (r) return r;
        { Timed t(c, RTX_K_ACCUM); if (lp) launch_accumulate_list(st, B.max_blocks, fb, P, c->accum_ptr(), lp->state); else launch_accumulate(st, B.max_blocks, fb, P, c->accum_ptr()); }
        HIPCHK(c, hipMemcpyAsync(c->pt.h_counters.as<uint32_t>() + (size_t)bi * ncnt, R.cnt, ncnt * 4, hipMemcpyDeviceToHost, st));
    }
    HIPCHK(c, hipEventRecord(c->ev.end, st));
    HIPCHK(c, hipGetLastError());
    aux_join.armed = false;
    c->pt.pending.active = true; c->pt.pending.ncnt = ncnt; c->pt.pending.nbatches = nbatches; c->pt.pending.G = G; c->pt.pending.mb = mb; c->pt.pending.nee = nee; c->pt.pending.nee1 = nee1;
    c->pt.pending.fused = tiny_fused; c->pt.pending.fused_bvh = fused_bvh;
    return RTX_OK;
}

void collect_timed(rtx_ctx* c) {
    for (const TimedLaunch& t : c->timed) { float m = 0.0f; if (hipEventElapsedTime(&m, t.a, t.b) == hipSuccess) c->stats.kernel_ms[t.cls] += m; }
    c->timed.clear();
}

int finish_render(rtx_ctx* c) {
    if (!c->pt.pending.active) return RTX_OK;
    c->pt.pending.active = false;
    const size_t ncnt = c->pt.pending.ncnt; const uint32_t nbatches = c->pt.pending.nbatches, G = c->pt.pending.G, mb = c->pt.pending.mb, nee = c->pt.pending.nee, nee1 = c->pt.pending.nee1;
    const bool fused = c->pt.pending.fused, fused_bvh = c->pt.pending.fused_bvh;
    HIPCHK(c, hipStreamSynchronize(c->stream));
    float ms = 0.0f;
    if (hipEventElapsedTime(&ms, c->ev.begin, c->ev.end) == hipSuccess) c->stats.render_ms += ms;
    collect_timed(c);
    if (!fused && !fused_bvh) { c->pt.pred_paths = 0; c->pt.pred_q.assign(mb, 0); c->pt.pred_s.assign((size_t)mb * nee1, 0); c->pt.pred_nee1 = nee1; }
    for (uint32_t bi = 0; bi < nbatches; bi++) {
        const uint32_t* h = c->pt.h_counters.as<uint32_t>() + (size_t)bi * ncnt;
        auto sumG = [&](size_t row) { uint64_t s = 0; for (uint32_t g = 0; g < G; g++) s += h[row * G + g]; return s; };
        if (!fused && !fused_bvh) {
            c->pt.pred_paths += sumG(0);
            for (uint32_t b = 0; b < mb; b++) { c->pt.pred_q[b] += sumG(b); for (uint32_t j = 0; j < nee1; j++) c->pt.pred_s[(size_t)b * nee1 + j] += sumG((size_t)(mb + 1) + (size_t)b * nee1 + j); }
        }
        const uint64_t prim = fused ? sumG((size_t)(mb + 1) + (size_t)mb * nee1) : sumG(0);
        c->stats.rays_primary += prim; c->stats.paths += prim;
        c->stats.primary_hits += fused ? sumG(0) : 0;
        for (uint32_t b = 1; b < mb; b++) c->stats.rays_extension += sumG(b);
        for (uint32_t b = 0; b < mb; b++) for (uint32_t j = 0; j < nee; j++) c->stats.rays_shadow += sumG((size_t)(mb + 1) + (size_t)b * nee1 + j);
    }
    c->stats.kernel_items[RTX_K_RAYGEN] = c->stats.paths;
    c->stats.kernel_items[RTX_K_BOUNCE] = fused ? c->stats.primary_hits + c->stats.rays_extension : fused_bvh ? c->stats.rays_primary + c->stats.rays_extension : 0;
    c->stats.kernel_items[RTX_K_TRACE] = (fused || fused_bvh) ? 0 : c->stats.rays_primary + c->stats.rays_extension;
    c->stats.kernel_items[RTX_K_SHADE] = (fused || fused_bvh) ? 0 : c->stats.rays_primary + c->stats.rays_extension;
    c->stats.kernel_items[RTX_K_SHADOW] = (fused || fused_bvh) ? 0 : c->stats.rays_shadow;
    c->stats.kernel_items[RTX_K_ACCUM] = c->stats.paths;
    return RTX_OK;
}
```

Before: 34590 Mrays/s.

## Slim shared-primary raygen: drop per-path hit records and hitmask writes

Result: faster. 35690 Mrays/s (median of 6 runs) (+3.2%).

```diff
diff --git a/royaltracer-dx_amd/csrc/rtx_dev_common.hpp b/royaltracer-dx_amd/csrc/rtx_dev_common.hpp
--- a/royaltracer-dx_amd/csrc/rtx_dev_common.hpp
+++ b/royaltracer-dx_amd/csrc/rtx_dev_common.hpp
@@ -67,5 +67,11 @@
     row0 += nk;
     return !(blockIdx.x >= nk || c >= nchunks);
 }
+__device__ __forceinline__ uint32_t deal_width(const DevFrame& f, uint32_t k) { return f.taper_levels ? taper_row_width(k, gridDim.x, f.taper_levels) : gridDim.x; }
+__device__ __forceinline__ uint32_t deal_row0(const DevFrame& f, uint32_t k, uint32_t period, uint32_t period_sum) {
+    uint32_t r = (k / period) * period_sum;
+    for (uint32_t j = 0; j < (k & (period - 1u)); j++) r += deal_width(f, j);
+    return r;
+}
 
 }
diff --git a/royaltracer-dx_amd/csrc/rtx_k_bounce_small.hpp b/royaltracer-dx_amd/csrc/rtx_k_bounce_small.hpp
--- a/royaltracer-dx_amd/csrc/rtx_k_bounce_small.hpp
+++ b/royaltracer-dx_amd/csrc/rtx_k_bounce_small.hpp
@@ -10,7 +10,7 @@
                                                          uint32_t* __restrict__ qrows ,
                                                          uint32_t* __restrict__ srows ,
                                                          const uint32_t* __restrict__ order ,
-                                                         const F4* __restrict__ prim_rec ) {
+                                                         PrimIn pin ) {
     extern __shared__ F4 lds[];
     __shared__ uint32_t s_cnt[1 + kMaxNee];
     DevFrame f = f_in;
@@ -69,12 +69,12 @@
             active = i < n;
             if (active) {
                 S.pid = myq[i];
-                const F4 e = p.hit[S.pid];
-                const uint32_t pl = f2u(e.x);
-                const F4 r0 = prim_rec[pl], r1 = prim_rec[(size_t)f.npl + pl], r2 = prim_rec[(size_t)2 * f.npl + pl], ro = prim_rec[(size_t)3 * f.npl];
-                S.s0 = f2u(e.y); S.s1 = f2u(e.z);
+                const uint32_t sl = __umulhi(S.pid, pin.div_mul) >> pin.div_shift, v = S.pid - sl * f.npl;
+                const uint32_t pl = f.list ? f.list[v >> 8] * (uint32_t)kBlock + (v & 255u) : v;
+                const F4 r0 = pin.rec[pl], r1 = pin.rec[(size_t)pin.npl + pl], r2 = pin.rec[(size_t)2 * pin.npl + pl], ro = pin.rec[(size_t)3 * pin.npl];
+                seed_sample(f2u(r2.w), f2u(r1.w), f.sample_first + sl, f.frame_seed, S.s0, S.s1);
                 S.o = mk3(ro.x, ro.y, ro.z); S.d = mk3(r0.x, r0.y, r0.z); S.thr = mk3(1.0f, 1.0f, 1.0f); S.prev_pdf = 1.0f;
-                sf.pos = mk3(r1.x, r1.y, r1.z); sf.normal = mk3(r2.x, r2.y, r2.z); sf.mat = f2u(r0.w); sf.near_hull = f2u(r1.w) != 0u;
+                sf.pos = mk3(r1.x, r1.y, r1.z); sf.normal = mk3(r2.x, r2.y, r2.z); sf.mat = f2u(r0.w) & 0x7FFFFFFFu; sf.near_hull = (f2u(r0.w) >> 31) != 0u;
                 prim = 0u;
             }
         } else if (HAVE_HIT) {
diff --git a/royaltracer-dx_amd/csrc/rtx_k_film.hpp b/royaltracer-dx_amd/csrc/rtx_k_film.hpp
--- a/royaltracer-dx_amd/csrc/rtx_k_film.hpp
+++ b/royaltracer-dx_amd/csrc/rtx_k_film.hpp
@@ -3,8 +3,8 @@
 
 namespace rtx {
 
-template <bool LIST>
-__global__ __launch_bounds__(kBlock) void k_accumulate(DevFrame f, DevPaths p, F4* __restrict__ accum, AdaptState ad) {
+template <bool LIST, bool SHARED>
+__global__ __launch_bounds__(kBlock) void k_accumulate(DevFrame f, DevPaths p, F4* __restrict__ accum, AdaptState ad, const unsigned long long* __restrict__ prim_hits) {
     const uint32_t stride = gridDim.x * kBlock;
     for (uint32_t pl = blockIdx.x * kBlock + threadIdx.x; pl < f.npl; pl += stride) {
         uint32_t x, y;
@@ -12,14 +12,18 @@
             uint32_t gi;
             if ((pl & 255u) == 0u && chunk_image_index(f, f.list[pl >> 8], gi)) ad.count[gi] = ad.count[gi] + f.batch_spp;
         }
-        if (!slot_to_pixel(f, real_slot<LIST>(f, pl), x, y)) continue;
+        const uint32_t rs = real_slot<LIST>(f, pl);
+        if (!slot_to_pixel(f, rs, x, y)) continue;
+        bool lit = true;
+        if constexpr (SHARED) lit = ((prim_hits[rs >> 6] >> (rs & 63u)) & 1ull) != 0ull;
         F4 a = accum[(size_t)y * f.width + x];
         F4 h = {0.0f, 0.0f, 0.0f, 0.0f};
         if constexpr (LIST) h = ad.half[(size_t)y * f.width + x];
         for (uint32_t s = 0; s < f.batch_spp; s++) {
             const size_t pid = (size_t)s * f.npl + pl;
             F4 r = {0.0f, 0.0f, 0.0f, 0.0f};
-            if (!p.hitmask || ((p.hitmask[pid >> 6] >> (pl & 63u)) & 1ull)) r = p.rad[pid];
+            if constexpr (SHARED) { if (lit) r = p.rad[pid]; }
+            else if (!p.hitmask || ((p.hitmask[pid >> 6] >> (pl & 63u)) & 1ull)) r = p.rad[pid];
             const f3 rv = mk3(r.x, r.y, r.z);
             if (finite3(rv)) {
                 a.x = a.x + rv.x; a.y = a.y + rv.y; a.z = a.z + rv.z; a.w = a.w + 1.0f;
diff --git a/royaltracer-dx_amd/csrc/rtx_k_raygen.hpp b/royaltracer-dx_amd/csrc/rtx_k_raygen.hpp
--- a/royaltracer-dx_amd/csrc/rtx_k_raygen.hpp
+++ b/royaltracer-dx_amd/csrc/rtx_k_raygen.hpp
@@ -130,46 +130,68 @@
     traverse_small<false>(sc, small, L, o, d, kTMinCam, valid ? kTMax : 0.0f, t, u, v, prim, sc.nsmall, keep);
     const bool hit = valid && prim != kMissPrim;
     const unsigned long long hm = __ballot(hit);
-    if (lane_id() == 0) { masks[pl >> 6] = keep; hits[pl >> 6] = hm; }
+    const unsigned long long vm = __ballot(valid);
+    if (lane_id() == 0) { masks[pl >> 6] = keep; hits[pl >> 6] = hm; hits[(f.npl >> 6) + (pl >> 6)] = vm; }
     if (pl == 0) rec[(size_t)3 * f.npl] = {cam.viewI[12], cam.viewI[13], cam.viewI[14], 0.0f};
     if (hit) {
         const Surf sf = surface(sc, o, d, t, u, v, prim);
-        rec[pl] = {d.x, d.y, d.z, u2f(sf.mat)};
-        rec[(size_t)f.npl + pl] = {sf.pos.x, sf.pos.y, sf.pos.z, u2f(sf.near_hull ? 1u : 0u)};
-        rec[(size_t)2 * f.npl + pl] = {sf.normal.x, sf.normal.y, sf.normal.z, 0.0f};
+        uint32_t h0, h1; seed_pixel(x, y, h0, h1);
+        rec[pl] = {d.x, d.y, d.z, u2f((sf.mat < 0x7FFFFFFFu ? sf.mat : 0x7FFFFFFFu) | (sf.near_hull ? 0x80000000u : 0u))};
+        rec[(size_t)f.npl + pl] = {sf.pos.x, sf.pos.y, sf.pos.z, u2f(h1)};
+        rec[(size_t)2 * f.npl + pl] = {sf.normal.x, sf.normal.y, sf.normal.z, u2f(h0)};
     }
 }
 
 template <bool LIST>
-__global__ __launch_bounds__(kBlock) void k_raygen_shared(DevFrame f, DevPaths p, uint32_t* __restrict__ queue, uint32_t* __restrict__ qcount, uint32_t* __restrict__ gencount,
-                                                          const unsigned long long* __restrict__ hits ) {
-    __shared__ uint32_t s_n[2];
-    if (threadIdx.x < 2) s_n[threadIdx.x] = 0;
+__global__ __launch_bounds__(kBlock) void k_raygen_shared(DevFrame f, uint32_t* __restrict__ queue, uint32_t* __restrict__ qcount, uint32_t* __restrict__ gencount,
+                                                          const unsigned long long* __restrict__ hits, uint32_t nblk) {
+    __shared__ unsigned long long s_hm[kBlock];
+    __shared__ uint32_t s_pid[kBlock], s_off[kBlock], s_wave[4], s_gen;
+    if (threadIdx.x == 0) s_gen = 0;
     __syncthreads();
     uint32_t* myq = queue + (size_t)blockIdx.x * f.qcap;
-    uint32_t generated = 0;
     const uint32_t nchunks = f.chunks_per_sample * f.batch_spp;
-    for (uint32_t k = 0, row0 = 0, c; row0 < nchunks; k++) {
-        if (!dealt_chunk(f, k, row0, nchunks, c)) continue;
-        const uint32_t sl = c / f.chunks_per_sample, cl = c - sl * f.chunks_per_sample;
-        const uint32_t pl = real_slot<LIST>(f, cl * kBlock + threadIdx.x);
-        const uint32_t pid = sl * f.npl + cl * kBlock + threadIdx.x;
-        uint32_t x = 0, y = 0;
-        if (slot_to_pixel(f, pl, x, y)) generated++;
-        const unsigned long long hm = hits[pl >> 6];
-        const bool hit = ((hm >> (pl & 63u)) & 1ull) != 0ull;
-        if (lane_id() == 0) p.hitmask[pid >> 6] = hm;
-        if (hit) {
-            if (f.max_bounces == 0u) p.rad[pid] = {0.0f, 0.0f, 0.0f, 0.0f};
-            uint32_t s0, s1; seed_init(x, y, f.sample_first + sl, f.frame_seed, s0, s1);
-            p.hit[pid] = {u2f(pl), u2f(s0), u2f(s1), 0.0f};
+    const uint32_t period = f.taper_levels ? 1u << (f.taper_levels - 1u) : 1u;
+    uint32_t period_sum = 0;
+    for (uint32_t j = 0; j < period; j++) period_sum += deal_width(f, j);
+    const uint32_t lane = threadIdx.x & 63u, wave = threadIdx.x >> 6;
+    uint32_t generated = 0, qn = 0;
+    for (uint32_t k0 = 0; deal_row0(f, k0, period, period_sum) < nchunks; k0 += 64u) {
+        const uint32_t k = k0 + (threadIdx.x >> 2);
+        uint32_t row0 = deal_row0(f, k, period, period_sum), c;
+        const bool dealt = dealt_chunk(f, k, row0, nchunks, c);
+        unsigned long long hm = 0ull;
+        uint32_t pid0 = 0;
+        if (dealt) {
+            const uint32_t sl = c / f.chunks_per_sample, cl = c - sl * f.chunks_per_sample;
+            const uint32_t v = cl * kBlock + (threadIdx.x & 3u) * 64u;
+            const uint32_t blk = real_slot<LIST>(f, v) >> 6;
+            hm = hits[blk];
+            generated += (uint32_t)__popcll(hits[nblk + blk]);
+            pid0 = sl * f.npl + v;
         }
-        const uint32_t slot = block_push(hit, &s_n[0]);
-        if (hit) myq[slot] = pid;
+        const uint32_t cnt = (uint32_t)__popcll(hm);
+        uint32_t inc = cnt;
+        for (uint32_t d = 1; d < 64u; d <<= 1) { const uint32_t y = __shfl_up(inc, d); if (lane >= d) inc += y; }
+        if (lane == 63u) s_wave[wave] = inc;
+        s_hm[threadIdx.x] = hm; s_pid[threadIdx.x] = pid0;
+        __syncthreads();
+        uint32_t before = 0, total = 0;
+        for (uint32_t w = 0; w < 4u; w++) { const uint32_t t = s_wave[w]; if (w < wave) before += t; total += t; }
+        s_off[threadIdx.x] = before + inc - cnt;
+        __syncthreads();
+        for (uint32_t i = wave; i < (uint32_t)kBlock; i += 4u) {
+            const unsigned long long m = s_hm[i];
+            if (!m) continue;
+            const uint32_t prefix = __builtin_amdgcn_mbcnt_hi((uint32_t)(m >> 32), __builtin_amdgcn_mbcnt_lo((uint32_t)m, 0u));
+            if ((m >> lane) & 1ull) myq[qn + s_off[i] + prefix] = s_pid[i] + lane;
+        }
+        qn += total;
+        __syncthreads();
     }
-    atomicAdd(&s_n[1], generated);
+    atomicAdd(&s_gen, generated);
     __syncthreads();
-    if (threadIdx.x == 0) { qcount[blockIdx.x] = s_n[0]; gencount[blockIdx.x] = s_n[1]; }
+    if (threadIdx.x == 0) { qcount[blockIdx.x] = qn; gencount[blockIdx.x] = s_gen; }
 }
 
 }
diff --git a/royaltracer-dx_amd/csrc/rtx_kernels.hip b/royaltracer-dx_amd/csrc/rtx_kernels.hip
--- a/royaltracer-dx_amd/csrc/rtx_kernels.hip
+++ b/royaltracer-dx_amd/csrc/rtx_kernels.hip
@@ -71,9 +71,9 @@
 void launch_primary_surface(hipStream_t st, const DevScene& sc, const DevFrame& f, const CameraGPU* cam, unsigned long long* masks, unsigned long long* hits, F4* rec) {
     hipLaunchKernelGGL(k_primary_surface, dim3(f.npl / kBlock), dim3(kBlock), trace_lds_bytes(sc), st, sc, sc.small, f, cam, masks, hits, rec);
 }
-void launch_raygen_shared(hipStream_t st, const DevFrame& f, const DevPaths& p, uint32_t* queue, uint32_t* qcount, uint32_t* gencount, const unsigned long long* hits) {
-    if (f.list) hipLaunchKernelGGL(k_raygen_shared<true>, dim3(f.nblocks), dim3(kBlock), 0, st, f, p, queue, qcount, gencount, hits);
-    else hipLaunchKernelGGL(k_raygen_shared<false>, dim3(f.nblocks), dim3(kBlock), 0, st, f, p, queue, qcount, gencount, hits);
+void launch_raygen_shared(hipStream_t st, const DevFrame& f, uint32_t* queue, uint32_t* qcount, uint32_t* gencount, const unsigned long long* hits, uint32_t rec_npl) {
+    if (f.list) hipLaunchKernelGGL(k_raygen_shared<true>, dim3(f.nblocks), dim3(kBlock), 0, st, f, queue, qcount, gencount, hits, rec_npl >> 6);
+    else hipLaunchKernelGGL(k_raygen_shared<false>, dim3(f.nblocks), dim3(kBlock), 0, st, f, queue, qcount, gencount, hits, rec_npl >> 6);
 }
 template <int V> using IntC = std::integral_constant<int, V>;
 template <bool V> using BoolC = std::integral_constant<bool, V>;
@@ -105,10 +105,11 @@
     });
 }
 void launch_bounce_small(hipStream_t st, const DevScene& sc, const DevFrame& f, const DevPaths& p, uint32_t bounce_first, uint32_t bounce_end,
-                         uint32_t* queue_a, uint32_t* queue_b, uint32_t* qrows, uint32_t* srows, const uint32_t* order, bool ring, const F4* prim_rec) {
+                         uint32_t* queue_a, uint32_t* queue_b, uint32_t* qrows, uint32_t* srows, const uint32_t* order, bool ring, const PrimIn* prim) {
     const bool lam = (f.flags & 1u) != 0u, have_hit = bounce_first == 0u;
-#define RTX_LAUNCH_BOUNCE(HH, LL, RR) hipLaunchKernelGGL((k_bounce_small<4, HH, LL, RR>), dim3(f.nblocks), dim3(kBlock), trace_lds_bytes(sc), st, sc, sc.small, f, p, bounce_first, bounce_end, queue_a, queue_b, qrows, srows, order, prim_rec)
-    if (have_hit && prim_rec) { if (lam) RTX_LAUNCH_BOUNCE(2, true, false); else RTX_LAUNCH_BOUNCE(2, false, false); }
+    const PrimIn pin = prim ? *prim : PrimIn{};
+#define RTX_LAUNCH_BOUNCE(HH, LL, RR) hipLaunchKernelGGL((k_bounce_small<4, HH, LL, RR>), dim3(f.nblocks), dim3(kBlock), trace_lds_bytes(sc), st, sc, sc.small, f, p, bounce_first, bounce_end, queue_a, queue_b, qrows, srows, order, pin)
+    if (have_hit && prim) { if (lam) RTX_LAUNCH_BOUNCE(2, true, false); else RTX_LAUNCH_BOUNCE(2, false, false); }
     else if (have_hit) { if (lam) RTX_LAUNCH_BOUNCE(1, true, false); else RTX_LAUNCH_BOUNCE(1, false, false); }
     else if (ring) { if (lam) RTX_LAUNCH_BOUNCE(0, true, true); else RTX_LAUNCH_BOUNCE(0, false, true); }
     else { if (lam) RTX_LAUNCH_BOUNCE(0, true, false); else RTX_LAUNCH_BOUNCE(0, false, false); }
@@ -216,11 +217,13 @@
 void launch_rs_p3_shade(hipStream_t st, const DevScene& sc, const DevFrame& f, const RsQ& q, uint32_t* const bufs[6], F4* accum) {
     hipLaunchKernelGGL(k_rs_p3_shade, dim3(q.G), dim3(kBlock), 0, st, sc, f, q, rs_bufs(bufs), accum);
 }
-void launch_accumulate(hipStream_t st, uint32_t max_blocks, const DevFrame& f, const DevPaths& p, F4* accum) {
-    hipLaunchKernelGGL(k_accumulate<false>, dim3(grid_for(f.npl, max_blocks)), dim3(kBlock), 0, st, f, p, accum, AdaptState{});
-}
-void launch_accumulate_list(hipStream_t st, uint32_t max_blocks, const DevFrame& f, const DevPaths& p, F4* accum, const AdaptState& ad) {
-    hipLaunchKernelGGL(k_accumulate<true>, dim3(grid_for(f.npl, max_blocks)), dim3(kBlock), 0, st, f, p, accum, ad);
+void launch_accumulate(hipStream_t st, uint32_t max_blocks, const DevFrame& f, const DevPaths& p, F4* accum, const unsigned long long* prim_hits) {
+    if (prim_hits) hipLaunchKernelGGL((k_accumulate<false, true>), dim3(grid_for(f.npl, max_blocks)), dim3(kBlock), 0, st, f, p, accum, AdaptState{}, prim_hits);
+    else hipLaunchKernelGGL((k_accumulate<false, false>), dim3(grid_for(f.npl, max_blocks)), dim3(kBlock), 0, st, f, p, accum, AdaptState{}, prim_hits);
+}
+void launch_accumulate_list(hipStream_t st, uint32_t max_blocks, const DevFrame& f, const DevPaths& p, F4* accum, const AdaptState& ad, const unsigned long long* prim_hits) {
+    if (prim_hits) hipLaunchKernelGGL((k_accumulate<true, true>), dim3(grid_for(f.npl, max_blocks)), dim3(kBlock), 0, st, f, p, accum, ad, prim_hits);
+    else hipLaunchKernelGGL((k_accumulate<true, false>), dim3(grid_for(f.npl, max_blocks)), dim3(kBlock), 0, st, f, p, accum, ad, prim_hits);
 }
 void launch_adaptive_error(hipStream_t st, const DevFrame& f, const F4* accum, const AdaptState& ad, float threshold, float dark_floor) {
     hipLaunchKernelGGL(k_adaptive_error, dim3(f.chunks_per_sample), dim3(kBlock), 0, st, f, accum, ad, threshold, dark_floor);
diff --git a/royaltracer-dx_amd/csrc/rtx_kernels.hpp b/royaltracer-dx_amd/csrc/rtx_kernels.hpp
--- a/royaltracer-dx_amd/csrc/rtx_kernels.hpp
+++ b/royaltracer-dx_amd/csrc/rtx_kernels.hpp
@@ -93,6 +93,13 @@
     uint8_t* oct_out; const uint8_t* oct_in; uint32_t* perm; uint32_t key_mode;
 };
 
+struct PrimIn { const F4* rec; uint32_t npl, div_mul, div_shift; };
+inline PrimIn prim_in(const F4* rec, uint32_t rec_npl, uint32_t d) {
+    uint32_t l = 0; while ((1ull << l) < d) l++;
+    const uint64_t m = (1ull << (31u + l)) / d + 1ull;
+    return PrimIn{rec, rec_npl, (uint32_t)m, l - 1u};
+}
+
 constexpr uint32_t kMaxMerge = 8;
 constexpr uint32_t kRsStreams = 7;
 constexpr uint32_t kRsOcc = 16;
@@ -118,10 +125,10 @@
 void launch_packet_masks(hipStream_t, const DevScene&, const DevFrame&, const CameraGPU* cam, unsigned long long* masks);
 void launch_raygen_trace_small(hipStream_t, const DevScene&, const DevFrame&, const DevPaths&, const CameraGPU* cam, uint32_t* queue, uint32_t* qcount, uint32_t* gencount, const unsigned long long* masks);
 void launch_primary_surface(hipStream_t, const DevScene&, const DevFrame&, const CameraGPU* cam, unsigned long long* masks, unsigned long long* hits, F4* rec);
-void launch_raygen_shared(hipStream_t, const DevFrame&, const DevPaths&, uint32_t* queue, uint32_t* qcount, uint32_t* gencount, const unsigned long long* hits);
+void launch_raygen_shared(hipStream_t, const DevFrame&, uint32_t* queue, uint32_t* qcount, uint32_t* gencount, const unsigned long long* hits, uint32_t rec_npl );
 void launch_bounce_small(hipStream_t, const DevScene&, const DevFrame&, const DevPaths&, uint32_t bounce_first, uint32_t bounce_end,
                          uint32_t* queue_a, uint32_t* queue_b, uint32_t* qrows, uint32_t* srows, const uint32_t* order, bool ring = true,
-                         const F4* prim_rec = nullptr);
+                         const PrimIn* prim = nullptr);
 void launch_bounce_bvh(hipStream_t, const DevScene&, const DevFrame&, const DevPaths&, uint32_t bounce_first, uint32_t bounce_end,
                        uint32_t* queue_a, uint32_t* queue_b, uint32_t* hitq, uint32_t* qrows, uint32_t* srows, const uint32_t* order);
 void launch_order_queues(hipStream_t, const uint32_t* qcount, uint32_t G, uint32_t* order);
@@ -149,9 +156,9 @@
 void launch_rs_p3_select(hipStream_t, const DevScene&, const DevFrame&, const RsQ&, const CameraGPU* cam, uint32_t* const bufs[6], uint32_t* shcnt, F4* key_a = nullptr, F4* key_b = nullptr);
 void launch_rs_p3_merge(hipStream_t, const DevScene&, const DevFrame&, const RsQ&, uint32_t* const bufs[6], uint32_t* shcnt);
 void launch_rs_p3_shade(hipStream_t, const DevScene&, const DevFrame&, const RsQ&, uint32_t* const bufs[6], F4* accum);
-void launch_accumulate(hipStream_t, uint32_t max_blocks, const DevFrame&, const DevPaths&, F4* accum);
+void launch_accumulate(hipStream_t, uint32_t max_blocks, const DevFrame&, const DevPaths&, F4* accum, const unsigned long long* prim_hits = nullptr);
 struct AdaptState { F4* half; uint32_t* count; uint32_t* flag; };
-void launch_accumulate_list(hipStream_t, uint32_t max_blocks, const DevFrame&, const DevPaths&, F4* accum, const AdaptState&);
+void launch_accumulate_list(hipStream_t, uint32_t max_blocks, const DevFrame&, const DevPaths&, F4* accum, const AdaptState&, const unsigned long long* prim_hits = nullptr);
 void launch_adaptive_error(hipStream_t, const DevFrame&, const F4* accum, const AdaptState&, float threshold, float dark_floor);
 void launch_adaptive_compact(hipStream_t, const DevFrame&, const AdaptState&, uint32_t max_spp, uint32_t* list, uint32_t* out5);
 struct DenoiseLevel { uint32_t width, height, tiles_x, step, normal_power_log2, first, last; float inv_sigma_plane, inv_sigma_color_s; };
diff --git a/royaltracer-dx_amd/csrc/rtx_math.hpp b/royaltracer-dx_amd/csrc/rtx_math.hpp
--- a/royaltracer-dx_amd/csrc/rtx_math.hpp
+++ b/royaltracer-dx_amd/csrc/rtx_math.hpp
@@ -92,6 +92,14 @@
     s0 = (y * 73856093u) ^ (x * 19349663u) ^ (s * 83492791u) ^ (frame_seed * 293803u);
     s1 = (x * 37623481u) ^ (y * 51964263u) ^ (s * 68250729u) ^ (frame_seed * 423977u);
 }
+RTX_HD void seed_pixel(uint32_t x, uint32_t y, uint32_t& h0, uint32_t& h1) {
+    h0 = (y * 73856093u) ^ (x * 19349663u);
+    h1 = (x * 37623481u) ^ (y * 51964263u);
+}
+RTX_HD void seed_sample(uint32_t h0, uint32_t h1, uint32_t s, uint32_t frame_seed, uint32_t& s0, uint32_t& s1) {
+    s0 = h0 ^ (s * 83492791u) ^ (frame_seed * 293803u);
+    s1 = h1 ^ (s * 68250729u) ^ (frame_seed * 423977u);
+}
 
 RTX_HD void sincos_(float x, float& sn, float& cs) {
     int j = (int)(x * 1.27323954473516f);
diff --git a/royaltracer-dx_amd/csrc/rtx_render.hip b/royaltracer-dx_amd/csrc/rtx_render.hip
--- a/royaltracer-dx_amd/csrc/rtx_render.hip
+++ b/royaltracer-dx_amd/csrc/rtx_render.hip
@@ -44,12 +44,12 @@
 int enqueue_tiny_fused(rtx_ctx* c, const FrameRun& R, const DevFrame& fb) {
     const hipStream_t st = R.st;
     uint32_t* gen_row = R.cnt + ((size_t)(R.mb + 1) + (size_t)R.mb * R.nee1) * R.G;
-    if (R.prim_rec) { Timed t(c, RTX_K_RAYGEN); launch_raygen_shared(st, fb, R.P, R.queue[0], R.Q(0), gen_row, (const unsigned long long*)c->pt.d_prim_hits.p); }
+    if (R.prim_rec) { Timed t(c, RTX_K_RAYGEN); launch_raygen_shared(st, fb, R.queue[0], R.Q(0), gen_row, (const unsigned long long*)c->pt.d_prim_hits.p, R.rec_npl); }
     else { Timed t(c, RTX_K_RAYGEN); launch_raygen_trace_small(st, c->dsc, fb, R.P, R.cam, R.queue[0], R.Q(0), gen_row, (const unsigned long long*)c->pt.d_pmask.p); }
     const uint32_t* order = nullptr;
     if (c->opt.lpt_order && R.G > 1) { launch_order_queues(st, R.Q(0), R.G, (uint32_t*)c->pt.d_order.p); order = (const uint32_t*)c->pt.d_order.p; }
-    DevFrame f0 = fb; f0.npl = R.rec_npl;
-    { Timed t(c, RTX_K_BOUNCE); launch_bounce_small(st, c->dsc, f0, R.P, 0, 1, R.queue[0], R.queue[1], R.Q(0), R.S(0, 0), order, false, R.prim_rec); }
+    const PrimIn prim = prim_in(R.prim_rec, R.rec_npl, fb.npl);
+    { Timed t(c, RTX_K_BOUNCE); launch_bounce_small(st, c->dsc, fb, R.P, 0, 1, R.queue[0], R.queue[1], R.Q(0), R.S(0, 0), order, false, R.prim_rec ? &prim : nullptr); }
     if (R.mb > 1) { Timed t(c, RTX_K_BOUNCE); launch_bounce_small(st, c->dsc, fb, R.P, 1, R.mb, R.queue[0], R.queue[1], R.Q(0), R.S(0, 0), order, c->opt.bounce_ring); }
     return RTX_OK;
 }
@@ -173,7 +173,7 @@
     if (R.stealing) HIPCHK(c, c->pt.d_heads.ensure(R.nheads * 4));
     HIPCHK(c, c->pt.d_pmask.ensure(((size_t)f_real.npl / 64 + 1) * 8));
     const bool shared_primary = tiny_fused && c->opt.shared_primary && !(p->flags & RTX_FLAG_JITTER);
-    if (shared_primary) { HIPCHK(c, c->pt.d_prim_rec.ensure(((size_t)f_real.npl * 3 + 1) * 16)); HIPCHK(c, c->pt.d_prim_hits.ensure(((size_t)f_real.npl / 64 + 1) * 8)); }
+    if (shared_primary) { HIPCHK(c, c->pt.d_prim_rec.ensure(((size_t)f_real.npl * 3 + 1) * 16)); HIPCHK(c, c->pt.d_prim_hits.ensure(((size_t)f_real.npl / 64 * 2 + 1) * 8)); }
     R.prim_rec = shared_primary ? (const F4*)c->pt.d_prim_rec.p : nullptr; R.rec_npl = f_real.npl;
     const size_t shn = qtot * R.nee1;
     HIPCHK(c, c->pt.d_sh_o.ensure(shn * 16)); HIPCHK(c, c->pt.d_sh_d.ensure(shn * 16)); HIPCHK(c, c->pt.d_sh_c.ensure(shn * 16));
@@ -184,7 +184,7 @@
     R.osort = c->opt.octant_sort && B.compact && !R.stealing;
     if (R.osort) { HIPCHK(c, c->pt.d_oct[0].ensure(qtot)); HIPCHK(c, c->pt.d_oct[1].ensure(qtot)); HIPCHK(c, c->pt.d_perm.ensure(qtot * 4)); }
     if (R.osort && c->opt.octant_sort == 2) { HIPCHK(c, hipMemsetAsync(c->pt.d_oct[0].p, 0, qtot, c->stream)); HIPCHK(c, hipMemsetAsync(c->pt.d_oct[1].p, 0, qtot, c->stream)); }
-    if (tiny_fused) { HIPCHK(c, c->pt.d_hitmask.ensure(((size_t)cap / 64 + 1) * 8)); P.hitmask = (unsigned long long*)c->pt.d_hitmask.p; }
+    if (tiny_fused && !shared_primary) { HIPCHK(c, c->pt.d_hitmask.ensure(((size_t)cap / 64 + 1) * 8)); P.hitmask = (unsigned long long*)c->pt.d_hitmask.p; }
     P.sh_o = (F4*)c->pt.d_sh_o.p; P.sh_d = (F4*)c->pt.d_sh_d.p; P.sh_c = (F4*)c->pt.d_sh_c.p;
     R.queue[0] = (uint32_t*)c->pt.d_queue[0].p; R.queue[1] = (uint32_t*)c->pt.d_queue[1].p;
     const uint32_t mb = R.mb, nee1 = R.nee1;
@@ -211,7 +211,8 @@
         if (c->opt.sample_interleave) while (fb.interleave < 4u && !((fb.batch_spp >> fb.interleave) & 1u)) fb.interleave++;
         r = tiny_fused ? enqueue_tiny_fused(c, R, fb) : fused_bvh ? enqueue_fused_bvh(c, R, fb) : enqueue_bounces(c, R, fb);
         if (r) return r;
-        { Timed t(c, RTX_K_ACCUM); if (lp) launch_accumulate_list(st, B.max_blocks, fb, P, c->accum_ptr(), lp->state); else launch_accumulate(st, B.max_blocks, fb, P, c->accum_ptr()); }
+        { Timed t(c, RTX_K_ACCUM); const unsigned long long* ph = shared_primary ? (const unsigned long long*)c->pt.d_prim_hits.p : nullptr;
+          if (lp) launch_accumulate_list(st, B.max_blocks, fb, P, c->accum_ptr(), lp->state, ph); else launch_accumulate(st, B.max_blocks, fb, P, c->accum_ptr(), ph); }
         HIPCHK(c, hipMemcpyAsync(c->pt.h_counters.as<uint32_t>() + (size_t)bi * ncnt, R.cnt, ncnt * 4, hipMemcpyDeviceToHost, st));
     }
     HIPCHK(c, hipEventRecord(c->ev.end, st));
```
